# PaulMullowney/hypre

Measured on AMD Instinct MI355X. Metric: BoomerAMG V-cycle DOF/s (256^3 7-pt Laplacian per GPU, l1-Jacobi V(1,1), fp64), higher is better.
Workload: dtype f64; 1 GPU; 256x256x256 7-pt Laplacian, 1 rank(s) 1x1x1, PMIS + ext+i(4) + l1-Jacobi V(1,1); transport=none, replicated_from_level=-1, coarse_tail_graph_from_level=-1, coarse_tail_graph_nodes=0, one_workgroup_tail_from_level=6, levels=9

## Files before the change

### hypre_amd/binding.py

```python
import ctypes as C
import os

import numpy as np

HERE = os.path.dirname(os.path.abspath(__file__))
LIB_PATH = os.environ.get("HYPRE_AMD_LIB") or os.path.join(HERE, "lib", "libhypre_amd.so")

HYPRE_MEMORY_HOST = 0
HYPRE_MEMORY_DEVICE = 1

Int = C.c_int
BigInt = C.c_longlong
Real = C.c_double
IntP = C.POINTER(C.c_int)
BigIntP = C.POINTER(C.c_longlong)
RealP = C.POINTER(C.c_double)


class HypreAmdError(RuntimeError):
    pass


class CSRMatrix(C.Structure):
    _fields_ = [("i", IntP), ("j", IntP), ("big_j", BigIntP), ("num_rows", Int), ("num_cols", Int),
# ... 19 lines not shown
class ParCSRMatrix(C.Structure):
    _fields_ = [("comm", Int), ("global_num_rows", BigInt), ("global_num_cols", BigInt),
                ("global_num_rownnz", BigInt), ("num_nonzeros", BigInt), ("d_num_nonzeros", Real),
                ("first_row_index", BigInt), ("first_col_diag", BigInt), ("last_row_index", BigInt),
                ("last_col_diag", BigInt), ("diag", C.POINTER(CSRMatrix)), ("offd", C.POINTER(CSRMatrix)),
                ("diagT", C.POINTER(CSRMatrix)), ("offdT", C.POINTER(CSRMatrix)), ("col_map_offd", BigIntP),
                ("device_col_map_offd", BigIntP), ("row_starts", BigInt * 2), ("col_starts", BigInt * 2),
                ("comm_pkg", C.POINTER(CommPkg)), ("comm_pkgT", C.POINTER(CommPkg)), ("owns_data", Int),
                ("rowindices", BigIntP), ("rowvalues", RealP), ("getrowactive", Int),
                ("assumed_partition", C.c_void_p), ("owns_assumed_partition", Int), ("proc_ordering", IntP),
                ("bdiag_size", Int), ("bdiaginv", RealP), ("bdiaginv_comm_pkg", C.c_void_p),
                ("soc_diag_j", IntP), ("soc_offd_j", IntP)]


class ParVector(C.Structure):
    _fields_ = [("comm", Int), ("global_size", BigInt), ("first_index", BigInt), ("last_index", BigInt),
                ("partitioning", BigInt * 2), ("actual_local_size", Int), ("local_vector", C.POINTER(Vector)),
                ("owns_data", Int), ("all_zeros", Int), ("assumed_partition", C.c_void_p)]


class IJMatrix(C.Structure):
    _fields_ = [("comm", Int), ("row_partitioning", BigInt * 2), ("col_partitioning", BigInt * 2),
                ("object_type", Int), ("object", C.c_void_p), ("translator", C.c_void_p),
                ("assumed_part", C.c_void_p), ("assemble_flag", Int), ("global_first_row", BigInt),
                ("global_first_col", BigInt), ("global_num_rows", BigInt), ("global_num_cols", BigInt),
                ("omp_flag", Int), ("print_level", Int)]


class IJVector(C.Structure):
    _fields_ = [("comm", Int), ("partitioning", BigInt * 2), ("num_components", Int), ("object_type", Int),
                ("object", C.c_void_p), ("translator", C.c_void_p), ("assumed_part", C.c_void_p),
                ("global_first_row", BigInt), ("global_num_rows", BigInt), ("print_level", Int)]


HYPRE_PARCSR = 5555


class IntArray(C.Structure):
    _fields_ = [("data", IntP), ("size", Int), ("memory_location", Int)]


class ErrorStruct(C.Structure):
    _fields_ = [("error_flag", Int), ("temp_error_flag", Int), ("print_to_memory", Int), ("verbosity", Int),
                ("memory", C.c_char_p), ("mem_sz", Int), ("msg_sz", Int)]


EXCHANGE_FN = C.CFUNCTYPE(C.c_int, C.c_void_p, C.c_int, IntP, C.POINTER(C.c_void_p), C.POINTER(C.c_size_t),
                          C.c_int, IntP, C.POINTER(C.c_void_p), C.POINTER(C.c_size_t), C.c_int, C.c_void_p)
ALLREDUCE_FN = C.CFUNCTYPE(C.c_int, C.c_void_p, RealP, C.c_int, C.c_int, C.c_void_p)
ALLGATHER_FN = C.CFUNCTYPE(C.c_int, C.c_void_p, C.c_void_p, C.c_void_p, C.c_size_t)
BARRIER_FN = C.CFUNCTYPE(C.c_int, C.c_void_p)
DESTROY_FN = C.CFUNCTYPE(None, C.c_void_p)


class CommOps(C.Structure):
    _fields_ = [("ctx", C.c_void_p), ("rank", C.c_int), ("size", C.c_int), ("exchange", EXCHANGE_FN),
                ("allreduce_sum", ALLREDUCE_FN), ("allgather", ALLGATHER_FN), ("barrier", BARRIER_FN),
                ("destroy", DESTROY_FN), ("device_buffers", C.c_int)]


CSRp = C.POINTER(CSRMatrix)
Vecp = C.POINTER(Vector)
ParCSRp = C.POINTER(ParCSRMatrix)
ParVecp = C.POINTER(ParVector)

PROTOTYPES = {
    "hypre_error_handler": (None, [C.c_char_p, Int, Int, C.c_char_p]),
    "HYPRE_GetError": (Int, []),
    "HYPRE_CheckError": (Int, [Int, Int]),
    "HYPRE_ClearError": (Int, [Int]),
    "HYPRE_ClearAllErrors": (Int, []),
    "HYPRE_GetErrorArg": (Int, []),
    "hypre_amd_LastErrorMessage": (C.c_char_p, []),
    "HYPRE_Initialize": (Int, []),
    "hypre_amd_HostCpuShare": (Int, []),
    "hypre_amd_SetHostThreads": (Int, [Int]),
    "HYPRE_Finalize": (Int, []),
    "HYPRE_SetMemoryLocation": (Int, [Int]),
    "HYPRE_GetMemoryLocation": (Int, [IntP]),
    "HYPRE_SetExecutionPolicy": (Int, [Int]),
    "HYPRE_GetExecutionPolicy": (Int, [IntP]),
    "hypre_amd_DeviceAvailable": (Int, []),
    "hypre_SetSyncCudaCompute": (Int, [Int]),
    "hypre_GetSyncCudaCompute": (Int, [IntP]),
    "hypre_SyncComputeStream": (Int, []),
    "hypre_amd_ByteCounters": (Int, [C.POINTER(C.c_double), C.POINTER(C.c_double), Int]),
    "hypre_amd_ComputeStream": (C.c_void_p, []),
    "hypre_amd_CommStream": (C.c_void_p, []),
    "hypre_amd_EventTimerStart": (Int, []),
    "hypre_amd_EventTimerStopMs": (Real, []),
    "hypre_MAlloc": (C.c_void_p, [C.c_size_t, Int]),
    "hypre_CAlloc": (C.c_void_p, [C.c_size_t, C.c_size_t, Int]),
    "hypre_Free": (None, [C.c_void_p, Int]),
    "hypre_Memcpy": (None, [C.c_void_p, C.c_void_p, C.c_size_t, Int, Int]),
    "hypre_Memset": (None, [C.c_void_p, Int, C.c_size_t, Int]),
    "hypre_GetExecPolicy1": (Int, [Int]),
    "hypre_GetExecPolicy2": (Int, [Int, Int]),
    "hypre_IntArrayCreate": (C.POINTER(IntArray), [Int]),
    "hypre_IntArrayInitialize_v2": (Int, [C.POINTER(IntArray), Int]),
    "hypre_IntArrayDestroy": (Int, [C.POINTER(IntArray)]),
    "hypre_amd_CommCreate": (Int, [C.POINTER(CommOps)]),
    "hypre_amd_CommDestroy": (Int, [Int]),
    "hypre_amd_RCCLGetUniqueId": (Int, [C.c_void_p]),
    "hypre_amd_CommCreateRCCL": (Int, [C.c_void_p, C.c_int, C.c_int]),
    "hypre_amd_CommCreateStreamStaged": (Int, [Int]),
    "hypre_MPI_Comm_rank": (Int, [Int, IntP]),
    "hypre_MPI_Comm_size": (Int, [Int, IntP]),
    "hypre_amd_CommSelfTest": (Int, [Int, Int]),
    "hypre_MPI_Barrier": (Int, [Int]),
    "hypre_amd_CommCounters": (Int, [BigIntP, BigIntP, Int]),
    "hypre_amd_CommSetTiming": (Int, [Int]),
    "hypre_amd_CommSetTag": (Int, [Int]),
    "hypre_amd_CommExposedTimes": (Int, [Int, IntP, IntP, RealP, RealP, RealP]),
    "hypre_amd_CommBytes": (Int, [C.POINTER(C.c_longlong), C.POINTER(C.c_longlong)]),
    "hypre_amd_ParCSRMatrixHaloInfo": (Int, [ParCSRp, C.POINTER(C.c_int), C.POINTER(C.c_int), C.POINTER(C.c_int), C.POINTER(C.c_int)]),
    "hypre_CSRMatrixCreate": (CSRp, [Int, Int, Int]),
    "hypre_CSRMatrixInitialize_v2": (Int, [CSRp, Int, Int]),
    "hypre_CSRMatrixInitialize": (Int, [CSRp]),
    "hypre_CSRMatrixDestroy": (Int, [CSRp]),
    "hypre_CSRMatrixSetRownnz": (Int, [CSRp]),
    "hypre_CSRMatrixMigrate": (Int, [CSRp, Int]),
    "hypre_CSRMatrixClone_v2": (CSRp, [CSRp, Int, Int]),
    "hypre_CSRMatrixTranspose": (Int, [CSRp, C.POINTER(CSRp), Int]),
    "hypre_CSRMatrixReorder": (Int, [CSRp]),
    "hypre_SeqVectorCreate": (Vecp, [Int]),
    "hypre_SeqMultiVectorCreate": (Vecp, [Int, Int]),
    "hypre_SeqVectorInitialize_v2": (Int, [Vecp, Int]),
    "hypre_SeqVectorInitialize": (Int, [Vecp]),
    "hypre_SeqVectorDestroy": (Int, [Vecp]),
    "hypre_SeqVectorMigrate": (Int, [Vecp, Int]),
    "hypre_SeqVectorCloneDeep_v2": (Vecp, [Vecp, Int]),
    "hypre_SeqVectorCloneDeep": (Vecp, [Vecp]),
    "hypre_CSRMatrixMatvecOutOfPlace": (Int, [Real, CSRp, Vecp, Real, Vecp, Vecp, Int]),
    "hypre_CSRMatrixMatvec": (Int, [Real, CSRp, Vecp, Real, Vecp]),
    "hypre_CSRMatrixMatvecT": (Int, [Real, CSRp, Vecp, Real, Vecp]),
    "hypre_CSRMatrixMatvecDevice": (Int, [Int, Real, CSRp, Vecp, Real, Vecp, Vecp, Int]),
    "hypre_CSRMatrixSpMVDevice": (Int, [Int, Real, CSRp, Vecp, Real, Vecp, Int]),
    "hypre_amd_CSRMatrixInvalidatePlan": (Int, [CSRp]),
    "hypre_amd_CSRMatrixVerifyPlan": (Int, [CSRp]),
    "hypre_amd_CSRMatrixSetImmutable": (Int, [CSRp, Int]),
    "hypre_amd_CSRMatrixPlanForm": (Int, [CSRp]),
    "hypre_amd_PlanTestFailAlloc": (Int, [Int, Int]),
    "hypre_amd_SetMixedPrecisionValues": (Int, [Int]),
    "hypre_amd_SpmvSetRowSlices": (Int, [Int]),
    "hypre_amd_SpmvSetFusedMultivectors": (Int, [Int]),
    "hypre_amd_SpmvFusedMultivectorLaunches": (Int, []),
    "hypre_amd_CSRMatrixPlanRowSlices": (Int, [CSRp, IntP, IntP]),
    "hypre_amd_CSRMatrixSortRows": (Int, [CSRp, Int]),
    "hypre_amd_SpmvSetBandPolicy": (Int, [Int, Int, Int]),
    "hypre_amd_SpmvSetVariant": (Int, [Int, Int]),
    "hypre_amd_CSRMatrixPlanInfo": (Int, [CSRp, IntP, IntP]),
    "hypre_amd_CSRMatrixPlanStaging": (Int, [CSRp, IntP, RealP]),
    "hypre_amd_SpmvSetValueCodes": (Int, [Int]),
    "hypre_amd_SpmvSetSliceForm": (Int, [Int]),
    "hypre_amd_CSRMatrixPlanSliceForm": (Int, [CSRp]),
    "hypre_amd_SpmvSetSliceClasses": (Int, [Int]),
    "hypre_amd_CSRMatrixPlanSliceClasses": (Int, [CSRp]),
    "hypre_amd_CSRMatrixPlanSliceClassHistogram": (Int, [CSRp, C.POINTER(Int), C.POINTER(Int), C.POINTER(BigInt)]),
    "hypre_amd_CSRMatrixPlanValueCodes": (Int, [CSRp]),
    "hypre_SeqVectorSetConstantValues": (Int, [Vecp, Real]),
    "hypre_SeqVectorCopy": (Int, [Vecp, Vecp]),
    "hypre_SeqVectorScale": (Int, [Real, Vecp]),
    "hypre_SeqVectorAxpy": (Int, [Real, Vecp, Vecp]),
    "hypre_SeqVectorAxpyz": (Int, [Real, Vecp, Real, Vecp, Vecp]),
    "hypre_SeqVectorInnerProd": (Real, [Vecp, Vecp]),
    "hypre_SeqVectorElmdivpy": (Int, [Vecp, Vecp, Vecp]),
    "hypre_SeqVectorElmdivpyMarked": (Int, [Vecp, Vecp, Vecp, IntP, Int]),
    "hypre_SeqVectorSetConstantValuesDevice": (Int, [Vecp, Real]),
    "hypre_SeqVectorScaleDevice": (Int, [Real, Vecp]),
    "hypre_SeqVectorAxpyDevice": (Int, [Real, Vecp, Vecp]),
    "hypre_SeqVectorAxpyzDevice": (Int, [Real, Vecp, Real, Vecp, Vecp]),
    "hypre_SeqVectorInnerProdDevice": (Real, [Vecp, Vecp]),
    "hypre_SeqVectorElmdivpyDevice": (Int, [Vecp, Vecp, Vecp, IntP, Int]),
    "hypreDevice_IVAXPY": (Int, [Int, RealP, RealP, RealP]),
    "hypreDevice_IVAXPYMarked": (Int, [Int, RealP, RealP, RealP, IntP, Int]),
    "hypreDevice_DiagScaleVector2": (Int, [Int, Int, RealP, RealP, Real, RealP, RealP, Int]),
    "hypre_ParCSRMatrixCreate": (ParCSRp, [Int, BigInt, BigInt, BigIntP, BigIntP, Int, Int, Int]),
    "hypre_ParCSRMatrixInitialize_v2": (Int, [ParCSRp, Int]),
    "hypre_ParCSRMatrixDestroy": (Int, [ParCSRp]),
    "hypre_ParCSRMatrixMigrate": (Int, [ParCSRp, Int]),
    "hypre_ParCSRMatrixClone_v2": (ParCSRp, [ParCSRp, Int, Int]),
    "hypre_ParCSRMatrixSetNumNonzeros": (Int, [ParCSRp]),
    "hypre_ParCSRMatrixSetDNumNonzeros": (Int, [ParCSRp]),
    "hypre_amd_ParCSRMatrixKeepTranspose": (Int, [ParCSRp]),
    "hypre_ParVectorCreate": (ParVecp, [Int, BigInt, BigIntP]),
    "hypre_ParMultiVectorCreate": (ParVecp, [Int, BigInt, BigIntP, Int]),
    "hypre_ParCSRDiagScaleVector": (Int, [ParCSRp, ParVecp, ParVecp]),
    "hypre_ParVectorInitialize_v2": (Int, [ParVecp, Int]),
    "hypre_ParVectorInitialize": (Int, [ParVecp]),
    "hypre_ParVectorDestroy": (Int, [ParVecp]),
    "hypre_ParVectorSetLocalSize": (Int, [ParVecp, Int]),
    "hypre_ParVectorMigrate": (Int, [ParVecp, Int]),
    "hypre_MatvecCommPkgCreate": (Int, [ParCSRp]),
    "hypre_MatvecCommPkgDestroy": (Int, [C.POINTER(CommPkg)]),
    "hypre_ParCSRCommPkgUpdateVecStarts": (Int, [C.POINTER(CommPkg), Int, Int, Int]),
    "hypre_ParCSRCommPkgCreate_core": (Int, [Int, BigIntP, BigInt, BigIntP, Int, Int, IntP, C.POINTER(IntP),
                                             C.POINTER(IntP), IntP, C.POINTER(IntP), C.POINTER(IntP),
                                             C.POINTER(IntP)]),
    "hypre_ParCSRCommHandleCreate_v2": (C.c_void_p, [Int, C.POINTER(CommPkg), Int, C.c_void_p, Int, C.c_void_p]),
    "hypre_ParCSRCommHandleCreate": (C.c_void_p, [Int, C.POINTER(CommPkg), C.c_void_p, C.c_void_p]),
    "hypre_ParCSRCommHandleDestroy": (Int, [C.c_void_p]),
    "hypre_ParCSRMatrixMatvecOutOfPlace": (Int, [Real, ParCSRp, ParVecp, Real, ParVecp, ParVecp]),
    "hypre_ParCSRMatrixMatvec": (Int, [Real, ParCSRp, ParVecp, Real, ParVecp]),
    "hypre_ParCSRMatrixMatvecT": (Int, [Real, ParCSRp, ParVecp, Real, ParVecp]),
    "hypre_ParCSRMatrixMatvecOutOfPlaceDevice": (Int, [Real, ParCSRp, ParVecp, Real, ParVecp, ParVecp]),
    "hypre_ParCSRMatrixMatvecTDevice": (Int, [Real, ParCSRp, ParVecp, Real, ParVecp]),
    "HYPRE_ParCSRMatrixMatvec": (Int, [Real, ParCSRp, ParVecp, Real, ParVecp]),
    "hypre_ParVectorSetConstantValues": (Int, [ParVecp, Real]),
    "hypre_ParVectorSetZeros": (Int, [ParVecp]),
    "hypre_ParVectorCopy": (Int, [ParVecp, ParVecp]),
    "hypre_ParVectorScale": (Int, [Real, ParVecp]),
    "hypre_ParVectorAxpy": (Int, [Real, ParVecp, ParVecp]),
    "hypre_ParVectorAxpyz": (Int, [Real, ParVecp, Real, ParVecp, ParVecp]),
    "hypre_ParVectorInnerProd": (Real, [ParVecp, ParVecp]),
    "hypre_ParVectorElmdivpy": (Int, [ParVecp, ParVecp, ParVecp]),
    "hypre_ParVectorElmdivpyMarked": (Int, [ParVecp, ParVecp, ParVecp, IntP, Int]),
    "GenerateLaplacian": (ParCSRp, [Int, BigInt, BigInt, BigInt, Int, Int, Int, Int, Int, Int, RealP]),
    "GenerateLaplacian27pt": (ParCSRp, [Int, BigInt, BigInt, BigInt, Int, Int, Int, Int, Int, Int, RealP]),
    "GenerateDifConv": (ParCSRp, [Int, BigInt, BigInt, BigInt, Int, Int, Int, Int, Int, Int, RealP]),
    "GenerateVarDifConv": (ParCSRp, [Int, BigInt, BigInt, BigInt, Int, Int, Int, Int, Int, Int, Real, C.POINTER(ParVecp)]),
    "GenerateRotate7pt": (ParCSRp, [Int, BigInt, BigInt, Int, Int, Int, Int, Real, Real]),
    "GenerateSysLaplacian": (ParCSRp, [Int, BigInt, BigInt, BigInt, Int, Int, Int, Int, Int, Int, Int, RealP, RealP]),
    "hypre_amd_CSRMatrixFromArrays": (CSRp, [Int, Int, Int, IntP, IntP, RealP, Int]),
    "hypre_amd_SeqVectorFromArray": (Vecp, [Int, RealP, Int]),
    "hypre_amd_SeqVectorToArray": (Int, [Vecp, RealP]),
    "hypre_amd_CopyToHost": (Int, [C.c_void_p, C.c_void_p, C.c_size_t, Int]),
    "hypre_amd_ParCSRMatrixFromArrays": (ParCSRp, [Int, BigInt, BigInt, BigIntP, BigIntP, Int, BigIntP, IntP, IntP,
                                                   RealP, IntP, IntP, RealP, Int]),
    "hypre_amd_ParVectorFromArray": (ParVecp, [Int, BigInt, BigIntP, RealP, Int]),
    "hypre_amd_ParVectorToArray": (Int, [ParVecp, RealP]),
    "HYPRE_IJMatrixRead": (Int, [C.c_char_p, Int, Int, C.POINTER(C.POINTER(IJMatrix))]),
    "HYPRE_IJMatrixPrint": (Int, [C.POINTER(IJMatrix), C.c_char_p]),
    "HYPRE_IJMatrixGetObject": (Int, [C.POINTER(IJMatrix), C.POINTER(C.c_void_p)]),
    "HYPRE_IJMatrixDestroy": (Int, [C.POINTER(IJMatrix)]),
    "hypre_ParCSRMatrixPrintIJ": (Int, [ParCSRp, Int, Int, C.c_char_p]),
    "HYPRE_IJVectorRead": (Int, [C.c_char_p, Int, Int, C.POINTER(C.POINTER(IJVector))]),
    "HYPRE_IJVectorPrint": (Int, [C.POINTER(IJVector), C.c_char_p]),
    "HYPRE_IJVectorGetObject": (Int, [C.POINTER(IJVector), C.POINTER(C.c_void_p)]),
    "HYPRE_IJVectorDestroy": (Int, [C.POINTER(IJVector)]),
    "hypre_amd_IJMatrixWrap": (C.POINTER(IJMatrix), [ParCSRp]),
    "hypre_amd_IJVectorWrap": (C.POINTER(IJVector), [ParVecp]),
}

_lib = None


def load_library(build_if_missing=False):
    global _lib
    if _lib is not None:
        return _lib
    if not os.path.exists(LIB_PATH):
        if build_if_missing:
            from . import build as _b
            _b.build()
        else:
            raise HypreAmdError("HIP library %s is missing — run `python -m hypre_amd.build` "
                                "(there is no fallback implementation)" % LIB_PATH)
    lib = C.CDLL(LIB_PATH, mode=C.RTLD_GLOBAL)
    from . import parcsr_ls_binding as _ls
    for table in (PROTOTYPES, _ls.PROTOTYPES):
        for name, (res, args) in table.items():
            fn = getattr(lib, name)
            fn.restype = res
            fn.argtypes = args
    _lib = lib
    return lib


class _LazyLib:
    def __getattr__(self, name):
        return getattr(load_library(), name)


lib = _LazyLib()


def check():
    L = load_library()
    flag = L.HYPRE_GetError()
    if flag:
        msg = L.hypre_amd_LastErrorMessage().decode()
        L.HYPRE_ClearAllErrors()
        raise HypreAmdError("hypre error flag 0x%x: %s" % (flag, msg))


def _ip(a):
    return a.ctypes.data_as(IntP)


def _bp(a):
    return a.ctypes.data_as(BigIntP)


def _rp(a):
    return a.ctypes.data_as(RealP)


def csr_from_scipy(A, location=HYPRE_MEMORY_DEVICE):
    A = A.tocsr()
    ii = np.ascontiguousarray(A.indptr, dtype=np.int32)
    jj = np.ascontiguousarray(A.indices, dtype=np.int32)
    aa = np.ascontiguousarray(A.data, dtype=np.float64)
    m = lib.hypre_amd_CSRMatrixFromArrays(A.shape[0], A.shape[1], int(A.nnz), _ip(ii), _ip(jj), _rp(aa), location)
    check()
    return m

# ... 104 lines not shown
```

### hypre_amd/csrc/internal.hpp

```cpp
#pragma once

#include <hip/hip_runtime.h>
#include <cstdio>
#include <cstdlib>
#include <cstring>
#include <cstdint>
#include <vector>

#include "HYPRE_amd_utilities.h"
#include "hypre_amd_seq_mv.h"
#include "hypre_amd_comm.h"
#include "hypre_amd_parcsr_mv.h"

#define HIP_CHECK(call)                                                          \
   do {                                                                          \
      hipError_t e_ = (call);                                                    \
      if (e_ != hipSuccess) {                                                    \
         char msg_[512];                                                         \
         snprintf(msg_, sizeof(msg_), "HIP error %d (%s) in %s", (int) e_,       \
                  hipGetErrorString(e_), #call);                                 \
         hypre_error_handler(__FILE__, __LINE__, HYPRE_ERROR_GENERIC, msg_);     \
      }                                                                          \
   } while (0)

#define HYPRE_AMD_REQUIRE_DEVICE(loc, what)                                      \
   do {                                                                          \
      if ((loc) != HYPRE_MEMORY_DEVICE) {                                        \
         hypre_error_w_msg(HYPRE_ERROR_GENERIC,                                  \
                           what ": operand is not in device memory; host "       \
                           "execution is not part of this library");             \
         return hypre_error_flag;                                                \
      }                                                                          \
   } while (0)

namespace hamd {

struct Handle
{
   bool                  device_ok      = false;
   bool                  device_probed  = false;
   hipStream_t           compute_stream = nullptr;
   hipStream_t           comm_stream    = nullptr;
   int                   sync_compute   = 1;
   HYPRE_MemoryLocation  memory_location = HYPRE_MEMORY_DEVICE;
   HYPRE_ExecutionPolicy exec_policy     = HYPRE_EXEC_DEVICE;
   double               *d_reduce      = nullptr;
   size_t                d_reduce_len  = 0;
   double               *h_reduce      = nullptr;
   int                   num_cus       = 256;
   int                   gs_threads    = 1;
   bool                  fp32_values   = false;
   double                bytes_csr     = 0.0;
   double                bytes_stream  = 0.0;
};
Handle &handle();
inline void account_bytes(double csr, double stream) { Handle &h = handle(); h.bytes_csr += csr; h.bytes_stream += stream; }
inline void account_bytes(double b) { account_bytes(b, b); }
const hypre_amd_CommOps *comm_ops(MPI_Comm comm);
bool    ensure_device();
int     host_cpu_share();
hipStream_t stream();
void    maybe_sync();
double *reduce_scratch(size_t n);

#ifndef HYPRE_AMD_SPMV_TILE_NNZ
#define HYPRE_AMD_SPMV_TILE_NNZ 2048
#endif
#ifndef HYPRE_AMD_SPMV_WG
#define HYPRE_AMD_SPMV_WG 256
#endif
constexpr int SPMV_TILE    = HYPRE_AMD_SPMV_TILE_NNZ;
constexpr int SPMV_MAXROW  = 1024;
constexpr int SPMV_THREADS = HYPRE_AMD_SPMV_WG;
static_assert(SPMV_TILE == 8 * SPMV_THREADS, "a lane streams two quads of the tile");

struct SpmvPlan
{
   const HYPRE_Int     *i = nullptr;
   const HYPRE_Int     *j = nullptr;
   const HYPRE_Complex *a = nullptr;
   int   num_rows = 0, num_cols = 0, nnz = 0;
   int   max_row_nnz = 0;
   int   max_tile_rows = 0;
   int   num_tiles = 0;
   int  *d_tile_row = nullptr;
   int  *d_tile_k   = nullptr;
   int  *d_tile_perm = nullptr;
   int   band = 0;
   int   prod_elems = 0;
   bool  tiled = false;
   hypre_CSRMatrix *AT = nullptr;
   hypre_CSRMatrix *Lstrict = nullptr;
   float *a32 = nullptr;
   unsigned char *d_codes = nullptr;
   double        *d_dict = nullptr, *d_dict32 = nullptr;
   int            ndict = 0;
   int       sl_w = 0, sl_rows = 0, sl_k = 0;
   int       sl_wc = 0, sl_wl = 0;
   int       sl_blocks = 0, sl_launch_units = 0;
   int      *d_sl_cnt = nullptr, *d_sl_desc = nullptr;
   int      *d_sl_k0 = nullptr, *d_sl_fp = nullptr;
   int      *d_sl_perm = nullptr;
   unsigned *d_sl_data = nullptr;
   unsigned char *d_sl_cls = nullptr;
   unsigned      *d_sl_tab = nullptr;
   int           *d_sl_toff = nullptr;
   int            sl_classes = 0;
   long long      sl_class_total = 0;
   bool has_slice_form() const { return d_sl_data != nullptr || d_sl_cls != nullptr; }
   int             rs_w = 0, rs_rows = 0, rs_kp = 0;
   int             rs_blocks = 0, rs_units = 0;
   int            *d_rs_desc = nullptr;
   int            *d_rs_perm = nullptr;
   int            *d_rs_hdr = nullptr;
   unsigned       *d_rs_meta = nullptr;
   double         *d_rs_val = nullptr;
   float          *d_rs_val32 = nullptr;
   unsigned       *d_rs_idx = nullptr;
   int            *d_xs_cnt = nullptr;
   int            *d_xs_desc = nullptr;
   unsigned short *d_lidx   = nullptr;
   int             xs_tiles = 0;
   int             xs_max_units = 0;
   int             xs_launch_units = 0;
   int            *d_tile_fp = nullptr;
   int            *h_stale = nullptr;
   int            *d_stale = nullptr;
   unsigned        launches = 0;
   unsigned long long checksum = 0;
   bool            has_checksum = false;
   bool            owned = false;
};
void mark_owned(const hypre_CSRMatrix *A, bool on = true);
bool is_owned(const hypre_CSRMatrix *A);
bool plan_verify(hypre_CSRMatrix *A);
enum PlanAllocSite { PLAN_SITE_TILES = 1, PLAN_SITE_XS = 2, PLAN_SITE_CODES = 3, PLAN_SITE_SLICE = 4, PLAN_SITE_ROWSLICE = 5, PLAN_SITE_SLICE_CLASSES = 6,
                     PLAN_SITE_MV_LEVELS = 7 };
bool plan_alloc(void **ptr, size_t bytes, int site);
void plan_free(void *ptr);
inline void verify_par_plans(hypre_ParCSRMatrix *A)
{
   if (!A) { return; }
   if (A->diag && A->diag->memory_location == HYPRE_MEMORY_DEVICE) { (void) plan_verify(A->diag); }
   if (A->offd && A->offd->memory_location == HYPRE_MEMORY_DEVICE) { (void) plan_verify(A->offd); }
}
unsigned long long device_csr_checksum(const int *Ai, const int *Aj, const double *Aa, int n, int nnz, hipStream_t s);
void bump_plan_generation();
constexpr int MATRIX_FP_WORDS = 16;
struct MatrixWatch
{
   unsigned long long *d_fp = nullptr;
   int *h_stale = nullptr, *d_stale = nullptr;
};
void watch_record(MatrixWatch &w, const hypre_CSRMatrix *A, bool with_values, hipStream_t s);
void watch_check(const MatrixWatch &w, const hypre_CSRMatrix *A, bool with_values, hipStream_t s);
bool watch_flagged(const MatrixWatch &w);
void watch_release(MatrixWatch &w);
int *take_stale_slot(int **device_view);
void give_stale_slot(int *slot);
void launch_matrix_fingerprint(const int *Ai, const int *Aj, const double *Aa, int n, int nnz, unsigned long long *fp, int *stale,
                               int record, hipStream_t s);
unsigned long long plan_generation();
bool plan_is_stale(const hypre_CSRMatrix *A);
void launch_build_fp(const HYPRE_Int *Aj, int nnz, int num_tiles, int *fp, hipStream_t s);
SpmvPlan *get_plan(hypre_CSRMatrix *A);
hypre_CSRMatrix *strict_lower_of(hypre_CSRMatrix *A);
void      drop_plan(hypre_CSRMatrix *A);
const float *fp32_values_of(hypre_CSRMatrix *A);
void      set_strict_lower(hypre_CSRMatrix *A, hypre_CSRMatrix *L);

enum SpmvOp
{
   OP_AXPBY   = 0,
   OP_JACOBI  = 1,
   OP_JACOBI_CF = 2,
   OP_TSGS    = 3,
   OP_JACOBI_MAP = 4,
   OP_AXPBY_DIV = 5,
   OP_RESID_RD = 6,
   OP_TSGS_FIRST = 7
};

struct SpmvArgs
{
   const HYPRE_Int     *Ai;
   const HYPRE_Int     *Aj;
   const HYPRE_Complex *Aa;
   const float         *Aa32;
   const unsigned char *Ac8;
   const double        *dict;
   int                  ndict;
   int                  dict_rounded;
   const HYPRE_Complex *x;
   const HYPRE_Complex *b;
   HYPRE_Complex       *y;
   HYPRE_Complex       *aux;
   const HYPRE_Complex *d;
   const HYPRE_Int     *marker;
   int                  marker_val;
   HYPRE_Complex        alpha, beta;
   HYPRE_Complex        scale2;
   int                  fill;
   int                  row_offset;
   int                  last_quad;
   int                  x_last;
   int                  reduce_w;
   int                  gather_t;
   int                  xcd_map;
   const int           *tile_perm;
   const int           *tile_fp;
   int                 *stale;
   const int           *rowmap;
   int                  variant;
   int                  use_rs;
   unsigned             rot;
   int                  nnz;
};
void spmv_default_flags(SpmvArgs &a);

void launch_spmv(const SpmvPlan *plan, const SpmvArgs &args, SpmvOp op, hipStream_t s);
bool spmv_with_scaled_quotient(hypre_CSRMatrix *M, const double *x, double *y, double w, const double *d, double *u);
bool launch_spmv_mv(const SpmvPlan *plan, const SpmvArgs &args, SpmvOp op, int nv, long xstride, long bstride, long ystride, long auxstride,
                    hipStream_t s);
struct MvStrides { long x, b, y, aux; };
void spmv_columns(HYPRE_Complex alpha, hypre_CSRMatrix *A, const double *x, size_t xstride, HYPRE_Complex beta, const double *b,
                  size_t bstride, double *y, size_t ystride, int nv);
void spmv_columns_jacobi(hypre_CSRMatrix *A, const double *f, size_t fstride, double w, const double *d, const double *u_in, size_t instride,
                         double *u_out, size_t outstride, int nv);
bool spmv_columns_scaled_quotient(hypre_CSRMatrix *M, const double *x, size_t xstride, double *y, size_t ystride, double w, const double *d,
                                  double *u, size_t ustride, int nv);
long &spmv_mv_launches();
bool &spmv_fused_multivectors();
void launch_spmv_rownnz(const HYPRE_Int *rownnz, int num_rownnz, const SpmvArgs &args, hipStream_t s);
void launch_spmv_allrows_update(int num_rows, const SpmvArgs &args, hipStream_t s);
bool device_value_codes(const double *Aa, size_t nnz, unsigned char **codes_out, double **dict_out, double **dict32_out, int *ndict_out,
                        hipStream_t s);
bool device_build_slice_form(SpmvPlan *p, const hypre_CSRMatrix *A, hipStream_t s);
bool device_build_row_slices(SpmvPlan *p, const hypre_CSRMatrix *A, hipStream_t s);
int  &spmv_row_slices();
bool &spmv_slice_classes();
bool &spmv_slice_form();
bool &spmv_value_codes();
void launch_build_tiles(const HYPRE_Int *Ai, int num_rows, int nnz, int num_tiles, int *d_tile_row,
                        int *d_tile_k, hipStream_t s);
void launch_build_xs(const HYPRE_Int *Aj, const int *d_tile_k, int num_tiles, int *xs_cnt, int *xs_desc, unsigned short *lidx,
                     hipStream_t s);
constexpr int SPMV_XS_SEGS = 48;
constexpr int SPMV_XS_CAP  = 4096;
int  device_max_row_nnz(const HYPRE_Int *Ai, int num_rows, hipStream_t s);
void sample_row_bands(const HYPRE_Int *Ai, const HYPRE_Int *Aj, int num_rows, int nsamples, int *host_out, hipStream_t s);

void launch_set(double *y, double v, size_t n, hipStream_t s);
void launch_copy(double *y, const double *x, size_t n, hipStream_t s);
void launch_scale(double *y, double a, size_t n, hipStream_t s);
void launch_axpy(double a, const double *x, double *y, size_t n, hipStream_t s);
void launch_axpyz(double a, const double *x, double b, const double *y, double *z, size_t n, hipStream_t s);
void launch_elmdivpy(const double *x, const double *d, double *y, const int *marker, int mval,
                     size_t n, hipStream_t s);
void launch_scaled_div(double w, const double *f, const double *d, double *u, const int *marker,
                       int mval, size_t n, hipStream_t s);
void launch_diag_first_scale(const int *Ai, const double *Aa, const double *y, double *x, size_t n, int nv, size_t ys, size_t xs, hipStream_t s);
void launch_scaled_recip(double w, const double *f, const double *d, double *z, size_t n, hipStream_t s);
void launch_diagscale2(const double *diag, const double *x, double beta, double *y, double *z,
                       int computeY, size_t n, hipStream_t s);
void launch_dot(const double *x, const double *y, size_t n, double *d_out, hipStream_t s);
void launch_gather(const double *x, const int *idx, double *out, size_t n, hipStream_t s);
void launch_scatter_add(const double *in, const int *idx, double *y, size_t n, hipStream_t s);
void launch_f64_to_f32(const double *x, float *y, size_t n, hipStream_t s);
void launch_transpose(const int *Ai, const int *Aj, const double *Aa, int nrows, int ncols, int nnz, int *Ti, int *tj, double *ta,
                      hipStream_t s);
void launch_scan_exclusive(int *data, int n, hipStream_t s);
void launch_sort_rows(const int *Ai, int *Aj, double *Aa, int n, int keep_first, hipStream_t s);
void preload_mc_kernels();
void prepare_mc_plan(hypre_CSRMatrix *A);
int  device_greedy_coloring(int n, const int *Ai, const int *Aj, const int *Ti, const int *Tj, int *color, int round_budget, hipStream_t s,
                            int *rounds_out = nullptr);
void device_color_order(int n, int C, const int *color, int **order_out, std::vector<int> &cstart, hipStream_t s);
void device_color_matrices(int n, int C, const int *color, const int *order, const std::vector<int> &cstart, const int *Ai, const int *Aj,
                           const double *Aa, int **ptr_out, int **Cj_out, double **Ca_out, std::vector<int> &slice0, std::vector<int> &slice_nnz,
                           hipStream_t s);
void launch_mc_diag(int n, const int *Ai, const double *Aa, double *d, hipStream_t s);
void launch_mc_rowinfo(int n, const int *order, const int *Ai, void *info, hipStream_t s);
void launch_mc_small_sweep_ahead(int num_colors, int direction, const int *cstart, const void *rowinfo, int nrows, const int *Aj,
                                 const double *Aa, const float *Aa32, int nnz_matrix, const double *f, const double *d, const int *marker,
                                 int marker_val, double w, double *u, int n, int nnz, int r_first, hipStream_t s);
void launch_mc_small_sweep(int num_colors, int direction, const int *cstart, const int *order, const int *Ai, const int *Aj,
                           const double *Aa, const float *Aa32, const double *f, const double *d, const int *marker, int marker_val,
                           double w, double *u, int n, int nnz, hipStream_t s);
void preload_cheby_kernels(); void preload_gs_kernels(); void preload_interp_kernels(); void preload_vector_kernels();
void preload_rap_kernels(); void preload_setup_kernels(); void preload_spmv_kernels();
void device_strength(int n, const int *Ai, const int *Aj, const double *Aa, double theta, double max_row_sum,
                     int **Si_out, int **Sj_out, int *nnz_out, hipStream_t s);
int  device_pmis(int n, const int *Si, const int *Sj, int snnz, unsigned seed, unsigned long long skip, int *CF, hipStream_t s);
int  device_coarse_numbering(int n, const int *CF, int *f2c, hipStream_t s);
bool device_l1_norms(int n, const int *Ai, const int *Aj, const double *Aa, int option, const int *cf, double *out, hipStream_t s);
bool device_rap(int nc, int ncP, int maxP, const int *Ri, const int *Rj, const double *Ra, const int *Ai, const int *Aj,
                const double *Aa, const int *Pi, const int *Pj, const double *Pa, int **Ci_out, int **Cj_out, double **Ca_out,
                int *nnz_out, hipStream_t s);
bool device_extpi(int n, const int *Ai, const int *Aj, const double *Aa, const int *Si, const int *Sj, const int *CF,
                  const int *f2c, double trunc_tol, int max_elmts, int first_rung, int **Pi_out, int **Pj_out, double **Pa_out,
                  int *nnz_out, hipStream_t s, int split = -1, int **Oi_out = nullptr, int **Oj_out = nullptr,
                  double **Oa_out = nullptr, int *onnz_out = nullptr);
void preload_dist_setup_kernels();
void device_extend_csr(int n, const int *Di, const int *Dj, const double *Da, const int *Oi, const int *Oj, const double *Oa, int ooff,
                       int ng, const int *Gi, const int *Gj, const double *Ga, int **Ei_out, int **Ej_out, double **Ea_out,
                       int *nnz_out, hipStream_t s);
void device_extract_rows(int filter, int tot, const int *d_elmts, const int *Di, const int *Dj, const double *Da,
                         const int *Oi, const int *Oj, const double *Oa, long long first_col, const long long *d_cmap, const int *CF,
                         std::vector<int> &hi, std::vector<long long> &hj, std::vector<double> &ha, hipStream_t s);
void device_extract_S_rows(int tot, const int *d_elmts, int n, const int *Si, const int *Sj, long long first_col, const long long *d_cmap,
                           const int *CFext, std::vector<int> &hi, std::vector<long long> &hj, hipStream_t s);
void device_split_strided(int n, int stride, int *len, int *nd, const int *sj, const double *sa, int split,
                          int **Di_out, int **Dj_out, double **Da_out, int *dnnz, int **Oi_out, int **Oj_out, double **Oa_out, int *onnz,
                          hipStream_t s);
void device_split_pattern(int n, const int *Si, const int *Sj, int split, int **Di_out, int **Dj_out, int *dnnz,
                          int **Oi_out, int **Oj_out, int *onnz, hipStream_t s);
void launch_mark_used(const int *j, size_t nnz, int *used, hipStream_t s);
void launch_renumber(int *j, size_t nnz, int split, const int *map, hipStream_t s);
void launch_gather_int(const int *x, const int *idx, int *out, size_t n, hipStream_t s);
bool device_l1_norms_blocks(int n, const int *Di, const int *Dj, const double *Da, const int *Oi, const int *Oj, const double *Oa,
                            int option, const int *cf, const int *cfo, double *out, hipStream_t s);
void device_strength_blocks(int n, const int *Di, const int *Dj, const double *Da, const int *Oi, const int *Oj, const double *Oa,
                            double theta, double max_row_sum, int **Si_out, int **Sj_out, int *nnz_out, hipStream_t s);
int  device_pmis_dist(int n, int nco, const int *Si, const int *Sj, int snnz, unsigned seed, unsigned long long skip,
                      hypre_ParCSRCommPkg *pkg, const int *d_elmts, const int *d_prev, MPI_Comm comm, int *CF, hipStream_t s);
bool device_rap_dist(bool direct, int nc, int square, int ncols_out, int maxP, int max_seed,
                     const int *Ri, const int *Rj, const double *Ra, const int *Ai, const int *Aj, const double *Aa,
                     const int *A2i, const int *A2j, const double *A2a, int a2_off, int nfine,
                     const int *Pi, const int *Pj, const double *Pa,
                     const int *Fi, const int *Fj, const int *Xi, const int *Xj, const double *Xa, int split,
                     int **Di_out, int **Dj_out, double **Da_out, int *dnnz, int **Oi_out, int **Oj_out, double **Oa_out, int *onnz,
                     hipStream_t s);
void launch_deinterleave(const double *in, double *out, int n, int nv, hipStream_t s);
void launch_interleave(const double *in, double *out, int n, int nv, hipStream_t s);
void launch_count_lower(const HYPRE_Int *Ai, const HYPRE_Int *Aj, int n, int *cnt, hipStream_t s);
void launch_fill_lower(const HYPRE_Int *Ai, const HYPRE_Int *Aj, const double *Aa, const HYPRE_Int *Li, HYPRE_Int *Lj,
                       double *La, int n, hipStream_t s);
void launch_pcg_update(double a, double na, const double *p, const double *s, double *x, double *r, size_t n,
                       double *d_out, hipStream_t stream);
void launch_pcg_direction(double beta, const double *s, double *p, size_t n, hipStream_t stream);
double global_sum(MPI_Comm comm, double v);
void   dev_allreduce_sum(MPI_Comm comm, double *d_buf, int n);
void   dev_global_sums(MPI_Comm comm, double *d_vals, int n, double *h_out);
void launch_scale_copy(double b, const double *x, double *y, size_t n, hipStream_t s);

}
```

### hypre_amd/csrc/seq_mv.cpp

```cpp
#include "internal.hpp"
#include <unordered_map>
#include <unordered_set>
#include <omp.h>
#include <algorithm>

using namespace hamd;

namespace hamd {

struct SpmvVariant { int variant; };
static SpmvVariant &spmv_variant()
{
   static SpmvVariant v = {-1};
   if (v.variant < 0)
   {
      const char *e = getenv("HYPRE_AMD_SPMV_VARIANT");
      v.variant = e ? atoi(e) : 2;
   }
   return v;
}

void spmv_default_flags(SpmvArgs &a)
{
   static int gt = -1, xcd = 8;
   if (gt < 0)
   {
      const char *e = getenv("HYPRE_AMD_SPMV_GT");
      gt = e ? atoi(e) : 1;
      e = getenv("HYPRE_AMD_SPMV_XCD");
      xcd = e ? atoi(e) : 8;
   }
   a.gather_t = gt; a.xcd_map = xcd;
   a.variant = spmv_variant().variant;
   { static int w = -1; if (w < 0) { const char *e = getenv("HYPRE_AMD_SPMV_REDUCE_W"); w = e ? atoi(e) : 0; } a.reduce_w = w; }
}

struct BandPolicy { int enabled, min_tiles, force; };
static BandPolicy &band_policy()
{
   static BandPolicy bp = {-1, 2048, 0};
   if (bp.enabled < 0)
   {
      const char *e = getenv("HYPRE_AMD_SPMV_BAND");
      bp.enabled = e ? atoi(e) : 1;
      if ((e = getenv("HYPRE_AMD_SPMV_BAND_MIN_TILES"))) { bp.min_tiles = atoi(e); }
      if ((e = getenv("HYPRE_AMD_SPMV_BAND_FORCE"))) { bp.force = atoi(e); }
   }
   return bp;
}

int g_fail_site = 0, g_fail_nth = 0;
bool plan_alloc(void **ptr, size_t bytes, int site)
{
   *ptr = nullptr;
   if (g_fail_site == site && g_fail_nth > 0 && --g_fail_nth == 0) { g_fail_site = 0; return false; }
   size_t free_b = 0, total_b = 0;
   if (bytes > ((size_t) 64 << 20))
   {
      if (hipMemGetInfo(&free_b, &total_b) != hipSuccess) { (void) hipGetLastError(); return false; }
      if (bytes > free_b / 2) { return false; }
   }
   if (hipMalloc(ptr, bytes ? bytes : 16) != hipSuccess) { (void) hipGetLastError(); *ptr = nullptr; return false; }
   return true;
}
void plan_free(void *ptr) { if (ptr) { HIP_CHECK(hipFree(ptr)); } }

static std::unordered_set<const hypre_CSRMatrix *> &owned_table()
{
   static std::unordered_set<const hypre_CSRMatrix *> t;
   return t;
}
void mark_owned(const hypre_CSRMatrix *A, bool on)
{
   if (!A) { return; }
   if (on) { owned_table().insert(A); } else { owned_table().erase(A); }
}
bool is_owned(const hypre_CSRMatrix *A) { return A && owned_table().count(A) != 0; }

static void build_band_placement(SpmvPlan *p, const hypre_CSRMatrix *A, hipStream_t s)
{
   const BandPolicy &bp = band_policy();
   if (!bp.enabled || p->num_tiles < bp.min_tiles || p->num_tiles < 8 || A->num_rows != A->num_cols) { return; }
   const int ns = 1024;
   std::vector<int> far((size_t) ns);
   sample_row_bands(A->i, A->j, A->num_rows, ns, far.data(), s);
   std::vector<int> sorted(far);
   std::sort(sorted.begin(), sorted.end());
   const int B = sorted[(size_t) ns / 2];
   int agree = 0;
   for (int f : far) { if (std::abs(f - B) * 50 <= B) { agree++; } }
   const long long rows_per_tile = std::max(1LL, (long long) A->num_rows / p->num_tiles);
   if (B <= 0 || agree * 10 < ns * 6 || 4LL * B > A->num_rows) { return; }
   if (!bp.force && (long long) B < 8 * 8 * rows_per_tile) { return; }
   std::vector<int> trow((size_t) p->num_tiles + 1);
   HIP_CHECK(hipMemcpyAsync(trow.data(), p->d_tile_row, sizeof(int) * ((size_t) p->num_tiles + 1), hipMemcpyDeviceToHost, s));
   HIP_CHECK(hipStreamSynchronize(s));
   std::vector<std::vector<int>> cls(8);
   for (int t = 0; t < p->num_tiles; t++)
   {
      const int c = (int) (((long long) (trow[(size_t) t] % B) * 8) / B);
      cls[(size_t) std::min(std::max(c, 0), 7)].push_back(t);
   }
   std::vector<int> perm((size_t) p->num_tiles, -1);
   std::vector<size_t> next(8, 0);
   std::vector<int> leftovers;
   for (int g = 0; g < p->num_tiles; g++)
   {
      const size_t c = (size_t) (g & 7);
      if (next[c] < cls[c].size()) { perm[(size_t) g] = cls[c][next[c]++]; }
   }
   for (size_t c = 0; c < 8; c++) { for (size_t k = next[c]; k < cls[c].size(); k++) { leftovers.push_back(cls[c][k]); } }
   size_t lo = 0;
   for (int g = 0; g < p->num_tiles; g++) { if (perm[(size_t) g] < 0) { perm[(size_t) g] = leftovers[lo++]; } }
   if (!plan_alloc((void **) &p->d_tile_perm, sizeof(int) * (size_t) p->num_tiles, PLAN_SITE_TILES)) { return; }
   HIP_CHECK(hipMemcpyAsync(p->d_tile_perm, perm.data(), sizeof(int) * (size_t) p->num_tiles, hipMemcpyHostToDevice, s));
   HIP_CHECK(hipStreamSynchronize(s));
   p->band = B;
}

constexpr int RP_CAP_HOST = 640;

static std::unordered_map<const hypre_CSRMatrix *, SpmvPlan *> &plan_table()
{
   static std::unordered_map<const hypre_CSRMatrix *, SpmvPlan *> t;
   return t;
}

static unsigned long long g_plan_generation = 1;
unsigned long long plan_generation() { return g_plan_generation; }
void bump_plan_generation() { g_plan_generation++; }

namespace {
struct StaleSlots
{
   std::vector<int *> pages;
   std::vector<int *> free_list;
   int used_in_last = 1024;
   int *take()
   {
      if (!free_list.empty()) { int *p = free_list.back(); free_list.pop_back(); *p = 0; return p; }
      if (used_in_last >= 1024)
      {
         int *page = nullptr;
         if (hipHostMalloc((void **) &page, sizeof(int) * 1024, hipHostMallocMapped) != hipSuccess) { (void) hipGetLastError(); return nullptr; }
         memset(page, 0, sizeof(int) * 1024);
         pages.push_back(page);
         used_in_last = 0;
      }
      return pages.back() + used_in_last++;
   }
   void give(int *p) { if (p) { free_list.push_back(p); } }
};
StaleSlots &stale_slots() { static StaleSlots s; return s; }
}

int *take_stale_slot(int **device_view)
{
   int *h = stale_slots().take();
   int *d = nullptr;
   if (h && hipHostGetDevicePointer((void **) &d, h, 0) != hipSuccess) { (void) hipGetLastError(); d = nullptr; }
   if (!d) { stale_slots().give(h); h = nullptr; }
   if (device_view) { *device_view = d; }
   return h;
}
void give_stale_slot(int *slot) { stale_slots().give(slot); }

void watch_record(MatrixWatch &w, const hypre_CSRMatrix *A, bool with_values, hipStream_t s)
{
   watch_release(w);
   w.h_stale = take_stale_slot(&w.d_stale);
   if (!w.h_stale) { return; }
   HIP_CHECK(hipMalloc((void **) &w.d_fp, sizeof(unsigned long long) * MATRIX_FP_WORDS));
   launch_matrix_fingerprint(A->i, A->j, with_values ? A->data : nullptr, A->num_rows, A->num_nonzeros, w.d_fp, w.d_stale, 1, s);
}
void watch_check(const MatrixWatch &w, const hypre_CSRMatrix *A, bool with_values, hipStream_t s)
{
   if (!w.d_fp) { return; }
   launch_matrix_fingerprint(A->i, A->j, with_values ? A->data : nullptr, A->num_rows, A->num_nonzeros, w.d_fp, w.d_stale, 0, s);
}
bool watch_flagged(const MatrixWatch &w) { return w.h_stale && __atomic_load_n(w.h_stale, __ATOMIC_RELAXED) != 0; }
void watch_release(MatrixWatch &w)
{
   if (w.d_fp) { HIP_CHECK(hipFree(w.d_fp)); }
   give_stale_slot(w.h_stale);
   w = MatrixWatch();
}

static void free_plan(SpmvPlan *p)
{
   if (!p) { return; }
   g_plan_generation++;
   if (p->d_tile_fp) { HIP_CHECK(hipFree(p->d_tile_fp)); }
   stale_slots().give(p->h_stale);
   if (p->d_tile_row) { HIP_CHECK(hipFree(p->d_tile_row)); }
   if (p->d_tile_k) { HIP_CHECK(hipFree(p->d_tile_k)); }
   if (p->d_tile_perm) { HIP_CHECK(hipFree(p->d_tile_perm)); }
   if (p->d_xs_cnt) { HIP_CHECK(hipFree(p->d_xs_cnt)); }
   if (p->d_xs_desc) { HIP_CHECK(hipFree(p->d_xs_desc)); }
   if (p->d_lidx) { HIP_CHECK(hipFree(p->d_lidx)); }
   if (p->a32) { HIP_CHECK(hipFree(p->a32)); }
   if (p->d_codes) { HIP_CHECK(hipFree(p->d_codes)); }
   if (p->d_dict) { HIP_CHECK(hipFree(p->d_dict)); }
   if (p->d_sl_cnt) { HIP_CHECK(hipFree(p->d_sl_cnt)); }
   if (p->d_sl_desc) { HIP_CHECK(hipFree(p->d_sl_desc)); }
   if (p->d_sl_k0) { HIP_CHECK(hipFree(p->d_sl_k0)); }
   if (p->d_sl_fp) { HIP_CHECK(hipFree(p->d_sl_fp)); }
   if (p->d_sl_perm) { HIP_CHECK(hipFree(p->d_sl_perm)); }
   if (p->d_sl_data) { HIP_CHECK(hipFree(p->d_sl_data)); }
   if (p->d_sl_cls) { HIP_CHECK(hipFree(p->d_sl_cls)); }
   if (p->d_sl_tab) { HIP_CHECK(hipFree(p->d_sl_tab)); }
   if (p->d_sl_toff) { HIP_CHECK(hipFree(p->d_sl_toff)); }
   for (void *q : {(void *) p->d_rs_desc, (void *) p->d_rs_perm, (void *) p->d_rs_hdr, (void *) p->d_rs_meta, (void *) p->d_rs_val,
                   (void *) p->d_rs_val32, (void *) p->d_rs_idx}) { plan_free(q); }
   if (p->AT) { hypre_CSRMatrixDestroy(p->AT); }
   if (p->Lstrict) { hypre_CSRMatrixDestroy(p->Lstrict); }
   delete p;
}

void drop_gs_schedule(const hypre_CSRMatrix *A);
void drop_mc_plan(const hypre_CSRMatrix *A);

void drop_plan(hypre_CSRMatrix *A)
{
   drop_gs_schedule(A);
   drop_mc_plan(A);
   auto &t = plan_table();
   auto it = t.find(A);
   if (it != t.end())
   {
      free_plan(it->second);
      t.erase(it);
   }
}

static bool build_tile_tables(SpmvPlan *p, const hypre_CSRMatrix *A, hipStream_t s)
{
   p->num_tiles = (int) (((long long) A->num_nonzeros + SPMV_TILE - 1) / SPMV_TILE);
   if (!plan_alloc((void **) &p->d_tile_row, sizeof(int) * (size_t) (p->num_tiles + 1), PLAN_SITE_TILES) ||
       !plan_alloc((void **) &p->d_tile_k, sizeof(int) * (size_t) (p->num_tiles + 1), PLAN_SITE_TILES))
   {
      plan_free(p->d_tile_row); plan_free(p->d_tile_k);
      p->d_tile_row = p->d_tile_k = nullptr;
      p->num_tiles = 0;
      return false;
   }
   p->prod_elems = SPMV_TILE + ((p->max_row_nnz + 3) & ~3) + 8;
   launch_build_tiles(A->i, A->num_rows, A->num_nonzeros, p->num_tiles, p->d_tile_row, p->d_tile_k, s);
   p->max_tile_rows = device_max_row_nnz(p->d_tile_row, p->num_tiles, s);
   p->h_stale = stale_slots().take();
   if (p->h_stale && hipHostGetDevicePointer((void **) &p->d_stale, p->h_stale, 0) != hipSuccess) { (void) hipGetLastError(); p->d_stale = nullptr; }
   if (!p->d_stale)
   {
      static int *sink = nullptr;
      if (!sink && hipMalloc((void **) &sink, sizeof(int)) != hipSuccess) { (void) hipGetLastError(); sink = nullptr; }
      if (sink) { HIP_CHECK(hipMemsetAsync(sink, 0, sizeof(int), s)); }
      p->d_stale = sink;
      stale_slots().give(p->h_stale); p->h_stale = nullptr;
   }
   return true;
}

static void build_staging(SpmvPlan *p, const hypre_CSRMatrix *A, hipStream_t s)
{
   if (spmv_value_codes() && p->d_stale) { device_value_codes(A->data, (size_t) A->num_nonzeros, &p->d_codes, &p->d_dict, &p->d_dict32, &p->ndict, s); }
   const int rs_mode = spmv_row_slices();
   if (!p->d_codes && (rs_mode >= 2 || (rs_mode == 1 && p->owned)) && device_build_row_slices(p, A, s)) { return; }
   if (!p->d_stale) { plan_free(p->d_codes); plan_free(p->d_dict); p->d_codes = nullptr; p->d_dict = p->d_dict32 = nullptr; p->ndict = 0; return; }
   const size_t nl = ((size_t) A->num_nonzeros + 15) & ~(size_t) 7;
   if (!plan_alloc((void **) &p->d_tile_fp, sizeof(int) * (size_t) p->num_tiles, PLAN_SITE_XS) ||
       !plan_alloc((void **) &p->d_xs_cnt, sizeof(int) * (size_t) p->num_tiles, PLAN_SITE_XS) ||
       !plan_alloc((void **) &p->d_xs_desc, sizeof(int) * (size_t) p->num_tiles * 2 * SPMV_XS_SEGS, PLAN_SITE_XS) ||
       !plan_alloc((void **) &p->d_lidx, sizeof(unsigned short) * nl, PLAN_SITE_XS))
   {
      plan_free(p->d_tile_fp); plan_free(p->d_xs_cnt); plan_free(p->d_xs_desc); plan_free(p->d_lidx);
      p->d_tile_fp = nullptr; p->d_xs_cnt = nullptr; p->d_xs_desc = nullptr; p->d_lidx = nullptr;
      plan_free(p->d_codes); plan_free(p->d_dict);
      p->d_codes = nullptr; p->d_dict = p->d_dict32 = nullptr; p->ndict = 0;
      return;
   }
   launch_build_fp(A->j, A->num_nonzeros, p->num_tiles, p->d_tile_fp, s);
   HIP_CHECK(hipMemsetAsync(p->d_lidx, 0, sizeof(unsigned short) * nl, s));
   launch_build_xs(A->j, p->d_tile_k, p->num_tiles, p->d_xs_cnt, p->d_xs_desc, p->d_lidx, s);
   std::vector<int> cnt((size_t) p->num_tiles);
   HIP_CHECK(hipMemcpyAsync(cnt.data(), p->d_xs_cnt, sizeof(int) * (size_t) p->num_tiles, hipMemcpyDeviceToHost, s));
   HIP_CHECK(hipStreamSynchronize(s));
   std::vector<int> cov;
   cov.reserve(cnt.size());
   for (int c : cnt) { if (c & 0xff) { p->xs_tiles++; p->xs_max_units = std::max(p->xs_max_units, c >> 8); cov.push_back(c >> 8); } }
   if (!cov.empty())
   {
      std::sort(cov.begin(), cov.end());
      static int pct = -1, verbose = 0;
      if (pct < 0)
      {
         const char *e = getenv("HYPRE_AMD_SPMV_XS_PCT");
         pct = e ? std::min(100, std::max(1, atoi(e))) : 99;
         verbose = getenv("HYPRE_AMD_PLAN_VERBOSE") != nullptr;
      }
      const int need = cov[(size_t) ((cov.size() - 1) * (size_t) pct / 100)];
      const int rows = p->max_tile_rows > 0 ? std::min(p->max_tile_rows, RP_CAP_HOST) : RP_CAP_HOST;
      const int other = 8 * (p->max_row_nnz > 12 ? ((std::min(rows, SPMV_THREADS) + 1) & ~1) : 0) + 4 * (rows + 4) + 64 +
                        (p->d_codes ? 8 * ((p->ndict + 1) & ~1) + 16 : 0);
      int units = p->xs_max_units;
      for (int wgs = 8; wgs >= 3; wgs--)
      {
         const int room = ((160 * 1024) / wgs) / 1280 * 1280;
         const int fit = (room - other) / 16;
         if (fit >= need) { units = std::min(fit, p->xs_max_units); break; }
      }
      p->xs_launch_units = std::max(units, need);
      if (verbose)
      {
         fprintf(stderr, "[plan] %d x %d, %d tiles: staged units p50 %d p90 %d p99 %d max %d -> launch %d (%d bytes of LDS)\n",
                 A->num_rows, A->num_cols, p->num_tiles, cov[cov.size() / 2], cov[(cov.size() - 1) * 9 / 10],
                 cov[(cov.size() - 1) * 99 / 100], cov.back(), p->xs_launch_units, 16 * p->xs_launch_units + other);
      }
   }
   p->prod_elems = std::max(p->prod_elems, 2 * p->xs_launch_units + 8);
   if (p->d_codes && spmv_slice_form()) { device_build_slice_form(p, A, s); }
}

SpmvPlan *get_plan(hypre_CSRMatrix *A)
{
   auto &t = plan_table();
   auto it = t.find(A);
   if (it != t.end())
   {
      SpmvPlan *p = it->second;
      const bool flagged = p->h_stale && __atomic_load_n(p->h_stale, __ATOMIC_RELAXED) != 0;
      if (!flagged && p->i == A->i && p->j == A->j && p->a == A->data && p->nnz == A->num_nonzeros &&
          p->num_rows == A->num_rows && p->num_cols == A->num_cols)
      {
         return p;
      }
      if (flagged)
      {
         hypre_error_w_msg(HYPRE_ERROR_GENERIC, "a kernel found its SpMV plan out of date (the matrix at this address is not the one the plan "
                                                "was built for, or its values changed without hypre_amd_CSRMatrixInvalidatePlan): the products "
                                                "since then are wrong; the plan is rebuilt");
         drop_gs_schedule(A);
         drop_mc_plan(A);
      }
      free_plan(p);
      t.erase(it);
   }
   SpmvPlan *p = new SpmvPlan();
   p->i = A->i; p->j = A->j; p->a = A->data;
   p->num_rows = A->num_rows; p->num_cols = A->num_cols; p->nnz = A->num_nonzeros;
   p->owned = is_owned(A);
   hipStream_t s = stream();
   if (A->num_rows > 0 && A->num_nonzeros > 0)
   {
      p->max_row_nnz = device_max_row_nnz(A->i, A->num_rows, s);
      const bool aligned = (((uintptr_t) A->j) & 15) == 0 && (((uintptr_t) A->data) & 15) == 0;
      p->tiled = aligned && p->max_row_nnz <= SPMV_MAXROW && build_tile_tables(p, A, s);
      if (p->tiled)
      {
         build_band_placement(p, A, s);
         if (spmv_variant().variant == 2) { build_staging(p, A, s); }
      }
      if (p->tiled && !p->owned)
      {
         p->checksum = device_csr_checksum(A->i, A->j, A->data, A->num_rows, A->num_nonzeros, s);
         p->has_checksum = true;
      }
   }
   t[A] = p;
   return p;
}

bool plan_verify(hypre_CSRMatrix *A)
{
   auto &t = plan_table();
   auto it = t.find(A);
   if (it == t.end()) { return true; }
   SpmvPlan *p = it->second;
   if (!p->has_checksum) { return true; }
   const bool same_arrays = p->i == A->i && p->j == A->j && p->a == A->data && p->nnz == A->num_nonzeros &&
                            p->num_rows == A->num_rows && p->num_cols == A->num_cols;
   if (same_arrays && device_csr_checksum(A->i, A->j, A->data, A->num_rows, A->num_nonzeros, stream()) == p->checksum) { return true; }
   drop_plan(A);
   return false;
}

bool &spmv_slice_form()
{
   static bool on = [] { const char *e = getenv("HYPRE_AMD_SPMV_SLICE_FORM"); return !(e && atoi(e) == 0); }();
   return on;
}

bool &spmv_slice_classes()
{
   static bool on = [] { const char *e = getenv("HYPRE_AMD_SPMV_SLICE_CLASSES"); return !(e && atoi(e) == 0); }();
   return on;
}

bool &spmv_fused_multivectors()
{
   static bool on = [] { const char *e = getenv("HYPRE_AMD_SPMV_FUSED_MV"); return !(e && atoi(e) == 0); }();
   return on;
}

bool &spmv_value_codes()
{
   static bool on = [] { const char *e = getenv("HYPRE_AMD_SPMV_VALUE_CODES"); return !(e && atoi(e) == 0); }();
   return on;
}

bool plan_is_stale(const hypre_CSRMatrix *A)
{
   auto &t = plan_table();
   auto it = t.find(A);
   return it != t.end() && it->second->h_stale && __atomic_load_n(it->second->h_stale, __ATOMIC_RELAXED) != 0;
}

const float *fp32_values_of(hypre_CSRMatrix *A)
{
   if (!A || A->num_nonzeros <= 0 || !A->data) { return nullptr; }
   SpmvPlan *p = get_plan(A);
   if (!p->a32)
   {
      HIP_CHECK(hipMalloc((void **) &p->a32, sizeof(float) * (((size_t) A->num_nonzeros + 3) & ~(size_t) 3)));
      launch_f64_to_f32(A->data, p->a32, (size_t) A->num_nonzeros, stream());
   }
   return p->a32;
}

void set_strict_lower(hypre_CSRMatrix *A, hypre_CSRMatrix *L)
{
   SpmvPlan *plan = get_plan(A);
   if (plan->Lstrict && plan->Lstrict != L) { hypre_CSRMatrixDestroy(plan->Lstrict); }
   plan->Lstrict = L;
}

hypre_CSRMatrix *strict_lower_of(hypre_CSRMatrix *A)
{
   SpmvPlan *plan = get_plan(A);
   if (plan->Lstrict) { return plan->Lstrict; }
   const int n = A->num_rows;
   hipStream_t s = stream();
   std::vector<int> cnt((size_t) std::max(n, 1)), off((size_t) n + 1, 0);
   int *d_cnt = hypre_TAlloc(int, (size_t) std::max(n, 1), HYPRE_MEMORY_DEVICE);
   launch_count_lower(A->i, A->j, n, d_cnt, s);
   HIP_CHECK(hipMemcpyAsync(cnt.data(), d_cnt, sizeof(int) * (size_t) n, hipMemcpyDeviceToHost, s));
   HIP_CHECK(hipStreamSynchronize(s));
   for (int i = 0; i < n; i++) { off[(size_t) i + 1] = off[(size_t) i] + cnt[(size_t) i]; }
   hypre_Free(d_cnt, HYPRE_MEMORY_DEVICE);
   hypre_CSRMatrix *L = hypre_CSRMatrixCreate(n, A->num_cols, off[(size_t) n]);
   hypre_CSRMatrixInitialize_v2(L, 0, HYPRE_MEMORY_DEVICE);
   hypre_TMemcpy(L->i, off.data(), HYPRE_Int, (size_t) n + 1, HYPRE_MEMORY_DEVICE, HYPRE_MEMORY_HOST);
   if (off[(size_t) n] > 0) { launch_fill_lower(A->i, A->j, A->data, L->i, L->j, L->data, n, s); }
   if (plan->owned) { mark_owned(L); }
   plan->Lstrict = L;
   return L;
}

bool spmv_with_scaled_quotient(hypre_CSRMatrix *M, const double *x, double *y, double w, const double *d, double *u)
{
   if (!M || M->num_rows <= 0 || M->num_nonzeros <= 0 || !d || !u || M->memory_location != HYPRE_MEMORY_DEVICE) { return false; }
   SpmvArgs a{};
   a.Ai = M->i; a.Aj = M->j; a.Aa = M->data; a.Aa32 = nullptr;
   a.x = x; a.b = nullptr; a.y = y; a.d = d; a.aux = u; a.marker = nullptr; a.marker_val = 0;
   a.alpha = 1.0; a.beta = 0.0; a.scale2 = w; a.fill = HYPRE_SPMV_FILL_WHOLE; a.row_offset = 0;
   spmv_default_flags(a);
   launch_spmv(get_plan(M), a, OP_AXPBY_DIV, stream());
   return true;
}
}

extern "C" HYPRE_Int hypre_amd_SpmvSetBandPolicy(HYPRE_Int enabled, HYPRE_Int min_tiles, HYPRE_Int force)
{
   hamd::BandPolicy &bp = hamd::band_policy();
   if (enabled >= 0) { bp.enabled = enabled; }
   if (min_tiles >= 0) { bp.min_tiles = min_tiles; }
   if (force >= 0) { bp.force = force; }
   return hypre_error_flag;
}

extern "C" HYPRE_Int hypre_amd_SpmvSetVariant(HYPRE_Int variant, HYPRE_Int unused)
{
   (void) unused;
   hamd::SpmvVariant &v = hamd::spmv_variant();
   if (variant >= 0) { v.variant = variant; }
   return hypre_error_flag;
}

extern "C" HYPRE_Int hypre_amd_SpmvSetValueCodes(HYPRE_Int on)
{
   if (on >= 0) { hamd::spmv_value_codes() = on != 0; }
   return hypre_error_flag;
}

extern "C" HYPRE_Int hypre_amd_SpmvSetSliceForm(HYPRE_Int on)
{
   if (on >= 0) { hamd::spmv_slice_form() = on != 0; }
   return hypre_error_flag;
}

extern "C" HYPRE_Int hypre_amd_SpmvSetSliceClasses(HYPRE_Int on)
{
   if (on >= 0) { hamd::spmv_slice_classes() = on != 0; }
   return hypre_error_flag;
}
extern "C" HYPRE_Int hypre_amd_CSRMatrixPlanSliceClasses(hypre_CSRMatrix *A)
{
   if (!A || A->memory_location != HYPRE_MEMORY_DEVICE) { return 0; }
   hamd::SpmvPlan *p = hamd::get_plan(A);
   return p->d_sl_cls ? p->sl_classes : 0;
}

extern "C" HYPRE_Int hypre_amd_CSRMatrixPlanSliceClassHistogram(hypre_CSRMatrix *A, HYPRE_Int *hist, HYPRE_Int *blocks, HYPRE_BigInt *total)
{
   if (!A || A->memory_location != HYPRE_MEMORY_DEVICE) { return 0; }
   hamd::SpmvPlan *p = hamd::get_plan(A);
   if (!p->d_sl_cls) { return 0; }
   std::vector<int> toff((size_t) p->sl_blocks + 1);
   HIP_CHECK(hipStreamSynchronize(hamd::stream()));
   HIP_CHECK(hipMemcpy(toff.data(), p->d_sl_toff, sizeof(int) * toff.size(), hipMemcpyDeviceToHost));
   if (hist)
   {
      for (int c = 0; c < 256; c++) { hist[c] = 0; }
      for (int b = 0; b < p->sl_blocks; b++) { hist[std::min(std::max(toff[(size_t) b + 1] - toff[(size_t) b], 0), 255)]++; }
   }
   if (blocks) { *blocks = p->sl_blocks; }
   if (total) { *total = (HYPRE_BigInt) p->sl_class_total; }
   return p->sl_classes;
}

extern "C" HYPRE_Int hypre_amd_SpmvSetRowSlices(HYPRE_Int mode)
{
   if (mode >= 0) { hamd::spmv_row_slices() = mode; }
   return hypre_error_flag;
}
extern "C" HYPRE_Int hypre_amd_CSRMatrixPlanRowSlices(hypre_CSRMatrix *A, HYPRE_Int *rows_per_block, HYPRE_Int *entries_per_lane)
{
   if (rows_per_block) { *rows_per_block = 0; }
   if (entries_per_lane) { *entries_per_lane = 0; }
   if (!A || A->memory_location != HYPRE_MEMORY_DEVICE) { return 0; }
   hamd::SpmvPlan *p = hamd::get_plan(A);
   if (!p->d_rs_val) { return 0; }
   if (rows_per_block) { *rows_per_block = p->rs_rows; }
   if (entries_per_lane) { *entries_per_lane = p->rs_kp; }
   return p->rs_w;
}

extern "C" HYPRE_Int hypre_amd_CSRMatrixPlanSliceForm(hypre_CSRMatrix *A)
{
   if (A->memory_location != HYPRE_MEMORY_DEVICE) { return 0; }
   hamd::SpmvPlan *p = hamd::get_plan(A);
   return p->has_slice_form() ? p->sl_w : 0;
}

extern "C" HYPRE_Int hypre_amd_CSRMatrixPlanValueCodes(hypre_CSRMatrix *A)
{
   if (A->memory_location != HYPRE_MEMORY_DEVICE) { return 0; }
   hamd::SpmvPlan *p = hamd::get_plan(A);
   return p->d_codes ? p->ndict : 0;
}

extern "C" HYPRE_Int hypre_amd_CSRMatrixPlanInfo(hypre_CSRMatrix *A, HYPRE_Int *num_tiles, HYPRE_Int *band)
{
   if (A->memory_location != HYPRE_MEMORY_DEVICE) { if (num_tiles) { *num_tiles = 0; } if (band) { *band = 0; } return 0; }
   hamd::SpmvPlan *p = hamd::get_plan(A);
   if (num_tiles) { *num_tiles = p->tiled ? p->num_tiles : 0; }
   if (band) { *band = p->band; }
   return p->d_tile_perm != nullptr;
}

extern "C" HYPRE_Int hypre_amd_CSRMatrixPlanStaging(hypre_CSRMatrix *A, HYPRE_Int *num_tiles, HYPRE_Real *mean_pieces)
{
   if (num_tiles) { *num_tiles = 0; }
   if (mean_pieces) { *mean_pieces = 0.0; }
   if (A->memory_location != HYPRE_MEMORY_DEVICE) { return 0; }
   hamd::SpmvPlan *p = hamd::get_plan(A);
   if (!p->tiled || !p->d_xs_cnt) { return 0; }
   std::vector<int> cnt((size_t) p->num_tiles);
   HIP_CHECK(hipStreamSynchronize(hamd::stream()));
   HIP_CHECK(hipMemcpy(cnt.data(), p->d_xs_cnt, sizeof(int) * (size_t) p->num_tiles, hipMemcpyDeviceToHost));
   long long staged = 0, pieces = 0;
   for (int c : cnt) { if (c & 0xff) { staged++; pieces += c & 0xff; } }
   if (num_tiles) { *num_tiles = p->num_tiles; }
   if (mean_pieces && staged) { *mean_pieces = (double) pieces / (double) staged; }
   return (HYPRE_Int) staged;
}

extern "C" HYPRE_Int hypre_amd_CSRMatrixSortRows(hypre_CSRMatrix *A, HYPRE_Int keep_first)
{
   HYPRE_AMD_REQUIRE_DEVICE(A->memory_location, "hypre_amd_CSRMatrixSortRows(A)");
   hamd::drop_plan(A);
   if (A->num_nonzeros > 0) { hamd::launch_sort_rows(A->i, A->j, A->data, A->num_rows, keep_first, hamd::stream()); }
   hamd::maybe_sync();
   return hypre_error_flag;
}

extern "C" HYPRE_Int hypre_amd_CSRMatrixInvalidatePlan(hypre_CSRMatrix *A)
{
   drop_plan(A);
   return hypre_error_flag;
}

extern "C" HYPRE_Int hypre_amd_CSRMatrixVerifyPlan(hypre_CSRMatrix *A)
{
   if (!A || A->memory_location != HYPRE_MEMORY_DEVICE) { return 1; }
   return hamd::plan_verify(A) ? 1 : 0;
}

extern "C" HYPRE_Int hypre_amd_CSRMatrixSetImmutable(hypre_CSRMatrix *A, HYPRE_Int on)
{
   if (!A) { hypre_error_in_arg(1); return hypre_error_flag; }
   if (hamd::is_owned(A) != (on != 0)) { drop_plan(A); hamd::mark_owned(A, on != 0); }
   return hypre_error_flag;
}

extern "C" HYPRE_Int hypre_amd_PlanTestFailAlloc(HYPRE_Int site, HYPRE_Int nth)
{
   const HYPRE_Int pending = hamd::g_fail_site ? hamd::g_fail_nth : 0;
   hamd::g_fail_site = nth > 0 ? site : 0;
   hamd::g_fail_nth = nth > 0 ? nth : 0;
   return pending;
}

extern "C" HYPRE_Int hypre_amd_SetMixedPrecisionValues(HYPRE_Int on)
{
   hamd::handle().fp32_values = on != 0;
   return hypre_error_flag;
}

extern "C" HYPRE_Int hypre_amd_CSRMatrixPlanForm(hypre_CSRMatrix *A)
{
   if (!A || A->memory_location != HYPRE_MEMORY_DEVICE) { return -1; }
   hamd::SpmvPlan *p = hamd::get_plan(A);
   if (!p->tiled) { return 0; }
   if (p->d_rs_val) { return 5; }
   if (!p->d_lidx) { return 1; }
   if (p->has_slice_form()) { return 4; }
   if (p->d_codes) { return 3; }
   return 2;
}

extern "C" {

hypre_CSRMatrix *hypre_CSRMatrixCreate(HYPRE_Int num_rows, HYPRE_Int num_cols, HYPRE_Int num_nonzeros)
{
   hypre_CSRMatrix *m = (hypre_CSRMatrix *) calloc(1, sizeof(hypre_CSRMatrix));
   mark_owned(m, false);
   m->num_rows = num_rows;
   m->num_cols = num_cols;
   m->num_nonzeros = num_nonzeros;
   m->num_rownnz = num_rows;
   m->owns_data = 1;
   m->memory_location = handle().memory_location;
   return m;
}

HYPRE_Int hypre_CSRMatrixInitialize_v2(hypre_CSRMatrix *m, HYPRE_Int bigInit, HYPRE_MemoryLocation loc)
{
   m->memory_location = loc;
   if (!m->data && m->num_nonzeros) { m->data = hypre_CTAlloc(HYPRE_Complex, m->num_nonzeros, loc); }
   if (!m->i) { m->i = hypre_CTAlloc(HYPRE_Int, m->num_rows + 1, loc); }
   if (bigInit)
   {
      if (!m->big_j && m->num_nonzeros) { m->big_j = hypre_CTAlloc(HYPRE_BigInt, m->num_nonzeros, loc); }
   }
   else
   {
      if (!m->j && m->num_nonzeros) { m->j = hypre_CTAlloc(HYPRE_Int, m->num_nonzeros, loc); }
   }
   return hypre_error_flag;
}

HYPRE_Int hypre_CSRMatrixInitialize(hypre_CSRMatrix *m)
{
   return hypre_CSRMatrixInitialize_v2(m, 0, m->memory_location);
}

HYPRE_Int hypre_CSRMatrixDestroy(hypre_CSRMatrix *m)
{
   if (!m) { return hypre_error_flag; }
   drop_plan(m);
   mark_owned(m, false);
   const HYPRE_MemoryLocation loc = m->memory_location;
   hypre_Free(m->rownnz, loc);
   if (m->owns_data)
   {
      hypre_Free(m->data, loc);
      hypre_Free(m->i, loc);
      hypre_Free(m->j, loc);
      hypre_Free(m->big_j, loc);
   }
   free(m);
   return hypre_error_flag;
}

HYPRE_Int hypre_CSRMatrixSetRownnz(hypre_CSRMatrix *m)
{
   const HYPRE_MemoryLocation loc = m->memory_location;
   const HYPRE_Int n = m->num_rows;
   std::vector<HYPRE_Int> hi;
   const HYPRE_Int *Ai = m->i;
   if (loc == HYPRE_MEMORY_DEVICE)
   {
      hi.resize((size_t) n + 1);
      hypre_TMemcpy(hi.data(), m->i, HYPRE_Int, n + 1, HYPRE_MEMORY_HOST, HYPRE_MEMORY_DEVICE);
      Ai = hi.data();
   }
   HYPRE_Int cnt = 0;
   for (HYPRE_Int r = 0; r < n; r++) { if (Ai[r + 1] > Ai[r]) { cnt++; } }
   hypre_Free(m->rownnz, loc);
   m->rownnz = nullptr;
   m->num_rownnz = cnt;
   if (cnt == 0 || cnt == n) { return hypre_error_flag; }
   std::vector<HYPRE_Int> list((size_t) cnt);
   cnt = 0;
   for (HYPRE_Int r = 0; r < n; r++) { if (Ai[r + 1] > Ai[r]) { list[(size_t) cnt++] = r; } }
   m->rownnz = hypre_TAlloc(HYPRE_Int, cnt, loc);
   hypre_TMemcpy(m->rownnz, list.data(), HYPRE_Int, cnt, loc, HYPRE_MEMORY_HOST);
   return hypre_error_flag;
}

static void migrate_array(void **p, size_t bytes, HYPRE_MemoryLocation from, HYPRE_MemoryLocation to)
{
   if (!*p) { return; }
   void *q = hypre_MAlloc(bytes ? bytes : 8, to);
   if (bytes) { hypre_Memcpy(q, *p, bytes, to, from); }
   hypre_Free(*p, from);
   *p = q;
}

HYPRE_Int hypre_CSRMatrixMigrate(hypre_CSRMatrix *A, HYPRE_MemoryLocation to)
{
   const HYPRE_MemoryLocation from = A->memory_location;
   if (from == to) { return hypre_error_flag; }
   drop_plan(A);
   migrate_array((void **) &A->i, sizeof(HYPRE_Int) * (size_t) (A->num_rows + 1), from, to);
   migrate_array((void **) &A->j, sizeof(HYPRE_Int) * (size_t) A->num_nonzeros, from, to);
   migrate_array((void **) &A->big_j, sizeof(HYPRE_BigInt) * (size_t) A->num_nonzeros, from, to);
   migrate_array((void **) &A->data, sizeof(HYPRE_Complex) * (size_t) A->num_nonzeros, from, to);
   if (A->rownnz) { migrate_array((void **) &A->rownnz, sizeof(HYPRE_Int) * (size_t) A->num_rownnz, from, to); }
   A->memory_location = to;
   return hypre_error_flag;
}

hypre_CSRMatrix *hypre_CSRMatrixClone_v2(hypre_CSRMatrix *A, HYPRE_Int copy_data, HYPRE_MemoryLocation loc)
{
   hypre_CSRMatrix *B = hypre_CSRMatrixCreate(A->num_rows, A->num_cols, A->num_nonzeros);
   hypre_CSRMatrixInitialize_v2(B, A->big_j != nullptr && A->j == nullptr, loc);
   const HYPRE_MemoryLocation src = A->memory_location;
   hypre_TMemcpy(B->i, A->i, HYPRE_Int, A->num_rows + 1, loc, src);
   if (A->j) { hypre_TMemcpy(B->j, A->j, HYPRE_Int, A->num_nonzeros, loc, src); }
   if (A->big_j && B->big_j) { hypre_TMemcpy(B->big_j, A->big_j, HYPRE_BigInt, A->num_nonzeros, loc, src); }
   if (copy_data && A->data) { hypre_TMemcpy(B->data, A->data, HYPRE_Complex, A->num_nonzeros, loc, src); }
   B->num_rownnz = A->num_rownnz;
   if (A->rownnz)
   {
      B->rownnz = hypre_TAlloc(HYPRE_Int, A->num_rownnz, loc);
      hypre_TMemcpy(B->rownnz, A->rownnz, HYPRE_Int, A->num_rownnz, loc, src);
   }
   return B;
}

HYPRE_Int hypre_CSRMatrixTranspose(hypre_CSRMatrix *A, hypre_CSRMatrix **AT_ptr, HYPRE_Int data)
{
   const HYPRE_MemoryLocation loc = A->memory_location;
   const HYPRE_Int nr = A->num_rows, nc = A->num_cols, nnz = A->num_nonzeros;
   if (loc == HYPRE_MEMORY_DEVICE)
   {
      hypre_CSRMatrix *AT = hypre_CSRMatrixCreate(nc, nr, nnz);
      const bool with_data = data && A->data;
      hypre_CSRMatrixInitialize_v2(AT, 0, loc);
      if (!with_data && AT->data) { hypre_Free(AT->data, loc); AT->data = nullptr; }
      launch_transpose(A->i, A->j, with_data ? A->data : nullptr, nr, nc, nnz, AT->i, AT->j, with_data ? AT->data : nullptr, stream());
      HIP_CHECK(hipStreamSynchronize(stream()));
      *AT_ptr = AT;
      return hypre_error_flag;
   }
   const HYPRE_Int *Ai = A->i, *Aj = A->j;
   const HYPRE_Complex *Aa = A->data;
   const bool with_data = data && A->data;
   std::vector<HYPRE_Int> ti((size_t) nc + 1, 0), tj((size_t) nnz);
   std::vector<HYPRE_Complex> ta(with_data ? (size_t) nnz : 0);
   int T = 1;
   if (nnz > (1 << 20))
   {
      T = std::min(omp_get_max_threads(), 16);
      while (T > 1 && (size_t) T * (size_t) nc > (size_t) 1 << 30) { T /= 2; }
   }
   if (T <= 1)
   {
// ... 528 lines not shown
```

### hypre_amd/csrc/spmv_kernels.hip

```cpp
#include "amg_internal.hpp"

namespace hamd {

typedef int    v4i __attribute__((ext_vector_type(4)));
typedef int    v2i __attribute__((ext_vector_type(2)));
typedef double v2d __attribute__((ext_vector_type(2)));
typedef float  v4f __attribute__((ext_vector_type(4)));

__device__ __forceinline__ double wave_sum64(double v)
{
#pragma unroll
   for (int off = 32; off > 0; off >>= 1) { v += __shfl_xor(v, off, 64); }
   return v;
}

template <int W>
__device__ __forceinline__ double subwave_sum(double v)
{
#pragma unroll
   for (int off = W / 2; off > 0; off >>= 1) { v += __shfl_xor(v, off, 64); }
   return v;
}

__device__ __forceinline__ bool fill_keep(int fill, int row, int col)
// ... 1229 lines not shown
{
   extern __shared__ __align__(16) unsigned char smem_raw[];
   double *xs = reinterpret_cast<double *>(smem_raw);
   const double *dictl = xs + stage_elems;
   unsigned *tabl = reinterpret_cast<unsigned *>(xs + stage_elems + ((p.ndict + 1) & ~1));

   const int block = block_of_workgroup(sl_perm, blocks);
   if (block < 0) { return; }

   const int tid = threadIdx.x, lane = tid & 63;
   const int wave = __builtin_amdgcn_readfirstlane(tid >> 6);
   constexpr int R = SPMV_THREADS / W;
   const int r = block * R + tid / W, sub = tid % W;
   SlLane<CLS, KP> me;
   sl_lane_load<CLS, W, KP>(me, st, p.Ai, block, wave, lane, tid, r, num_rows);
   const RowOps ops = load_row_ops<OP>(p, max(min(r, num_rows - 1), 0));
   const XPieces pc = wave_x_pieces(sl_desc, block, wave);
   const int k0 = sl_k0[block], k1b = sl_k0[block + 1], fp_plan = sl_fp[block];
   asm volatile("" :: "s"(sl_desc), "s"(sl_k0), "s"(sl_fp), "s"(CLS ? (const void *) st.toff : (const void *) st.data), "s"(st.tab), "s"(p.Ai) : "memory");
   stage_x_pieces<1>(p.x, 0, xs, 0, pc, lane);
   sl_lane_stage<CLS, KP>(me, st, wave, lane, tabl);
   stage_value_table(p.dict, p.ndict, dictl, wave, lane);
   const int q0 = min(max(k0, 0), nnz - 1), q1 = min(max(k0, 0) + 1, nnz - 1);
   const int fc0 = p.Aj[q0], fc1 = p.Aj[q1];
   const int ck = min(max(min(k0 + 8 * (int) ((4u * p.rot + (unsigned) wave) & 511u) + (lane & 7), k1b - 1), 0), nnz - 1);
   const double ckv = p.Aa[ck];
   const unsigned ckc = p.Ac8[ck];
   __syncthreads();

   const int mylen = sl_lane_words<CLS, W, KP>(me, tid, tabl);
   double sum = 0.0;
#pragma unroll
   for (int j = 0; j < KP; j++)
   {
      const unsigned code = (me.cw[j >> 2] >> (8 * (j & 3))) & 0xffu;
      const unsigned li = (me.lw[j >> 1] >> (16 * (j & 1))) & 0xffffu;
      {
#pragma clang fp contract(off)
         const double pr = dictl[code] * xs[li];
         if (j < mylen) { sum = sum + pr; }
      }
   }
   if (W == 2) { sum += __shfl_xor(sum, 1, 64); }
   {
      bool off = __double_as_longlong(dictl[ckc]) != __double_as_longlong(p.dict_rounded ? (double) (float) ckv : ckv);
      if (tid == 0) { off = off || fp_plan != plan_fingerprint(fc0, fc1) || me.rs != k0; }
      if (off) { mark_stale(p); }
   }
   if (r < num_rows && sub == 0) { row_epilogue<OP>(p, r, sum, ops); }
}
template <int OP, int W, int KP>
__global__ __launch_bounds__(SPMV_THREADS)
void spmv_sl_kernel(SpmvArgs p, const int *__restrict__ sl_cnt, const int *__restrict__ sl_desc, const int *__restrict__ sl_k0,
                    const int *__restrict__ sl_fp, const int *__restrict__ sl_perm, const unsigned *__restrict__ sl_data,
                    int blocks, int num_rows, int nnz, int stage_elems)
{
   const SlStream st = {sl_data, nullptr, nullptr, nullptr};
   spmv_sl_body<OP, W, KP, false>(p, sl_desc, sl_k0, sl_fp, sl_perm, st, blocks, num_rows, nnz, stage_elems);
}
template <int OP, int W, int KP>
__global__ __launch_bounds__(SPMV_THREADS)
void spmv_sl_kernel_cls(SpmvArgs p, const int *__restrict__ sl_desc, const int *__restrict__ sl_k0, const int *__restrict__ sl_fp,
                        const int *__restrict__ sl_perm, const unsigned char *__restrict__ sl_cls, const unsigned *__restrict__ sl_tab,
                        const int *__restrict__ sl_toff, int blocks, int num_rows, int nnz, int stage_elems)
{
   const SlStream st = {nullptr, sl_cls, sl_tab, sl_toff};
   spmv_sl_body<OP, W, KP, true>(p, sl_desc, sl_k0, sl_fp, sl_perm, st, blocks, num_rows, nnz, stage_elems);
}

template <int NV, int W, int KP, bool CLS, int OP>
__device__ __forceinline__
void spmv_sl_mv_body(const SpmvArgs &p, const int *__restrict__ sl_desc, const int *__restrict__ sl_k0,
                     const int *__restrict__ sl_fp, const int *__restrict__ sl_perm, const SlStream &st,
                     int blocks, int num_rows, int nnz, int stage_elems, MvStrides ms)
{
   extern __shared__ __align__(16) unsigned char smem_raw[];
   double *xs = reinterpret_cast<double *>(smem_raw);
   const double *dictl = xs + (size_t) NV * stage_elems;
   unsigned *tabl = reinterpret_cast<unsigned *>(xs + (size_t) NV * stage_elems + ((p.ndict + 1) & ~1));

   const int block = block_of_workgroup(sl_perm, blocks);
   if (block < 0) { return; }

   const int tid = threadIdx.x, lane = tid & 63;
   const int wave = __builtin_amdgcn_readfirstlane(tid >> 6);
   constexpr int R = SPMV_THREADS / W;
   const int r = block * R + tid / W, sub = tid % W;
   SlLane<CLS, KP> me;
   sl_lane_load<CLS, W, KP>(me, st, p.Ai, block, wave, lane, tid, r, num_rows);
   MvOps<NV> ops;
   mv_load_ops<NV, OP>(ops, p, max(min(r, num_rows - 1), 0), ms);
   const XPieces pc = wave_x_pieces(sl_desc, block, wave);
   const int k0 = sl_k0[block], k1b = sl_k0[block + 1], fp_plan = sl_fp[block];
   asm volatile("" :: "s"(sl_desc), "s"(sl_k0), "s"(sl_fp), "s"(CLS ? (const void *) st.toff : (const void *) st.data), "s"(st.tab), "s"(p.Ai) : "memory");
   sl_lane_stage<CLS, KP>(me, st, wave, lane, tabl);
   stage_x_pieces<NV>(p.x, ms.x, xs, stage_elems, pc, lane);
   stage_value_table(p.dict, p.ndict, dictl, wave, lane);
   const int q0 = min(max(k0, 0), nnz - 1), q1 = min(max(k0, 0) + 1, nnz - 1);
   const int fc0 = p.Aj[q0], fc1 = p.Aj[q1];
   const int ck = min(max(min(k0 + 8 * (int) ((4u * p.rot + (unsigned) wave) & 511u) + (lane & 7), k1b - 1), 0), nnz - 1);
   const double ckv = p.Aa[ck];
   const unsigned ckc = p.Ac8[ck];
   __syncthreads();

   const int mylen = sl_lane_words<CLS, W, KP>(me, tid, tabl);
   double sum[NV];
#pragma unroll
   for (int v = 0; v < NV; v++) { sum[v] = 0.0; }
#pragma unroll
   for (int j = 0; j < KP; j++)
   {
      const unsigned code = (me.cw[j >> 2] >> (8 * (j & 3))) & 0xffu;
      const unsigned li = (me.lw[j >> 1] >> (16 * (j & 1))) & 0xffffu;
      const double a = dictl[code];
#pragma unroll
      for (int v = 0; v < NV; v++)
      {
#pragma clang fp contract(off)
         const double pr = a * xs[v * stage_elems + li];
         if (j < mylen) { sum[v] = sum[v] + pr; }
      }
   }
   if (W == 2)
   {
#pragma unroll
      for (int v = 0; v < NV; v++) { sum[v] += __shfl_xor(sum[v], 1, 64); }
   }
   {
      bool off = __double_as_longlong(dictl[ckc]) != __double_as_longlong(ckv);
      if (tid == 0) { off = off || fp_plan != plan_fingerprint(fc0, fc1) || me.rs != k0; }
      if (off) { mark_stale(p); }
   }
   if (r < num_rows && sub == 0) { mv_epilogue<NV, OP>(p, r, sum, ops, ms); }
}
template <int NV, int W, int KP, int OP>
__global__ __launch_bounds__(SPMV_THREADS)
void spmv_sl_mv_kernel(SpmvArgs p, const int *__restrict__ sl_desc, const int *__restrict__ sl_k0,
                       const int *__restrict__ sl_fp, const int *__restrict__ sl_perm, const unsigned *__restrict__ sl_data,
                       int blocks, int num_rows, int nnz, int stage_elems, MvStrides ms)
{
   const SlStream st = {sl_data, nullptr, nullptr, nullptr};
   spmv_sl_mv_body<NV, W, KP, false, OP>(p, sl_desc, sl_k0, sl_fp, sl_perm, st, blocks, num_rows, nnz, stage_elems, ms);
}
template <int NV, int W, int KP, int OP>
__global__ __launch_bounds__(SPMV_THREADS)
void spmv_sl_mv_kernel_cls(SpmvArgs p, const int *__restrict__ sl_desc, const int *__restrict__ sl_k0, const int *__restrict__ sl_fp,
                           const int *__restrict__ sl_perm, const unsigned char *__restrict__ sl_cls, const unsigned *__restrict__ sl_tab,
                           const int *__restrict__ sl_toff, int blocks, int num_rows, int nnz, int stage_elems, MvStrides ms)
{
   const SlStream st = {nullptr, sl_cls, sl_tab, sl_toff};
   spmv_sl_mv_body<NV, W, KP, true, OP>(p, sl_desc, sl_k0, sl_fp, sl_perm, st, blocks, num_rows, nnz, stage_elems, ms);
}

__global__ void sl_block_starts_kernel(const int *__restrict__ Ai, int num_rows, int R, int blocks, int *__restrict__ k0)
{
   const int b = blockIdx.x * blockDim.x + threadIdx.x;
   if (b <= blocks) { k0[b] = Ai[min((long long) b * R, (long long) num_rows)]; }
}
__global__ void sl_fp_kernel(const int *__restrict__ Aj, const int *__restrict__ k0, int blocks, int nnz, int *__restrict__ fp)
{
   const int b = blockIdx.x * blockDim.x + threadIdx.x;
   if (b >= blocks) { return; }
   const int q0 = min(max(k0[b], 0), nnz - 1), q1 = min(max(k0[b], 0) + 1, nnz - 1);
   fp[b] = plan_fingerprint(Aj[q0], Aj[q1]);
}
template <int W>
__global__ __launch_bounds__(SPMV_THREADS)
void sl_pack_kernel(const int *__restrict__ Ai, const unsigned char *__restrict__ codes, const unsigned short *__restrict__ lidx,
                    int num_rows, int kper, int wc, int wl, unsigned *__restrict__ data)
{
   constexpr int R = SPMV_THREADS / W;
   const int block = blockIdx.x, tid = threadIdx.x, lane = tid & 63, wave = tid >> 6;
   const int r = block * R + tid / W, sub = tid % W;
   const int rs = r < num_rows ? Ai[r] : 0, re = r < num_rows ? Ai[r + 1] : 0;
   unsigned *out = data + ((size_t) (block * 4 + wave) * (size_t) (wc + wl)) * 64 + lane;
   for (int w = 0; w < wc; w++)
   {
      unsigned word = 0;
      for (int q = 0; q < 4; q++)
      {
         const int j = 4 * w + q, k = rs + sub + j * W;
         if (j < kper && k < re) { word |= (unsigned) codes[k] << (8 * q); }
      }
      out[w * 64] = word;
   }
   for (int w = 0; w < wl; w++)
   {
      unsigned word = 0;
      for (int q = 0; q < 2; q++)
      {
         const int j = 2 * w + q, k = rs + sub + j * W;
         if (j < kper && k < re) { word |= (unsigned) lidx[k] << (16 * q); }
      }
      out[(wc + w) * 64] = word;
   }
}

constexpr int SL_CLASS_CAP = 255;
static inline int sl_stage_elems_of(int units, bool classes) { return classes ? std::max(2 * units + 8, SPMV_THREADS) : 2 * units + 8; }
template <int W>
__device__ inline void sl_lane_tuple(const int *__restrict__ Ai, const unsigned *__restrict__ data, int num_rows, int wc, int wl,
                                     int block, int tid, unsigned *tup)
{
   constexpr int R = SPMV_THREADS / W;
   const int lane = tid & 63, wave = tid >> 6, t = tid / W, sub = tid % W;
   const int r = block * R + t;
   const int rs = r < num_rows ? Ai[r] : 0, re = r < num_rows ? Ai[r + 1] : 0;
   const int mylen = max((re - rs - sub + W - 1) / W, 0);
   const unsigned *sd = data + ((size_t) (block * 4 + wave) * (size_t) (wc + wl)) * 64 + lane;
   tup[0] = (unsigned) mylen;
   for (int w = 0; w < wc; w++) { tup[1 + w] = sd[w * 64]; }
   for (int w = 0; w < wl; w++)
   {
      const unsigned v = sd[(wc + w) * 64];
      const unsigned lo = 2 * w < mylen ? ((v & 0xffffu) - (unsigned) t) & 0xffffu : 0u;
      const unsigned hi = 2 * w + 1 < mylen ? ((v >> 16) - (unsigned) t) & 0xffffu : 0u;
      tup[1 + wc + w] = lo | (hi << 16);
   }
   for (int w = 1 + wc + wl; w < 16; w++) { tup[w] = 0u; }
}
template <int W>
__global__ __launch_bounds__(SPMV_THREADS)
void sl_classify_kernel(const int *__restrict__ Ai, const unsigned *__restrict__ data, int num_rows, int wc, int wl,
                        unsigned char *__restrict__ cls, int *__restrict__ ncls)
{
   __shared__ unsigned tupS[SPMV_THREADS][17];
   __shared__ int leader;
   const int block = blockIdx.x, tid = threadIdx.x;
   unsigned tup[16];
   sl_lane_tuple<W>(Ai, data, num_rows, wc, wl, block, tid, tup);
   for (int w = 0; w < 16; w++) { tupS[tid][w] = tup[w]; }
   int mine = -1, round = 0;
   while (true)
   {
      if (tid == 0) { leader = SPMV_THREADS; }
      __syncthreads();
      if (mine < 0) { atomicMin(&leader, tid); }
      __syncthreads();
      const int L = leader;
      if (L == SPMV_THREADS || round == SL_CLASS_CAP) { if (L != SPMV_THREADS) { round = SL_CLASS_CAP + 1; } break; }
      if (mine < 0)
      {
         bool eq = true;
         for (int w = 0; w < 16; w++) { eq = eq && tupS[L][w] == tup[w]; }
         if (eq) { mine = round; }
      }
      round++;
      __syncthreads();
   }
   cls[(size_t) block * SPMV_THREADS + tid] = (unsigned char) max(mine, 0);
   if (tid == 0) { ncls[block] = round; }
}
template <int W>
__global__ __launch_bounds__(SPMV_THREADS)
void sl_class_table_kernel(const int *__restrict__ Ai, const unsigned *__restrict__ data, int num_rows, int wc, int wl, int kper,
                           const unsigned char *__restrict__ cls, const int *__restrict__ toff, unsigned *__restrict__ tab)
{
   __shared__ int first[256];
   const int block = blockIdx.x, tid = threadIdx.x;
   first[tid] = SPMV_THREADS;
   __syncthreads();
   const int c = cls[(size_t) block * SPMV_THREADS + tid];
   atomicMin(&first[c], tid);
   __syncthreads();
   if (first[c] != tid) { return; }
   unsigned tup[16];
   sl_lane_tuple<W>(Ai, data, num_rows, wc, wl, block, tid, tup);
   unsigned *out = tab + ((size_t) toff[block] + (size_t) c) * (size_t) kper;
   for (int w = 0; w < kper; w++) { out[w] = tup[w]; }
}
static_assert(SPMV_THREADS == 256, "a class byte per lane of a 256-lane block; sl_class_table_kernel's first[]");

static bool device_build_slice_classes(SpmvPlan *p, const hypre_CSRMatrix *A, hipStream_t s)
{
   const int blocks = p->sl_blocks, kper = p->sl_k, wc = p->sl_wc, wl = p->sl_wl, n = A->num_rows;
   unsigned char *d_cls = nullptr;
   int *d_ncls = nullptr, *d_toff = nullptr;
   unsigned *d_tab = nullptr;
   auto fail = [&]() -> bool
   {
      HIP_CHECK(hipStreamSynchronize(s));
      for (void *q : {(void *) d_cls, (void *) d_ncls, (void *) d_toff, (void *) d_tab}) { plan_free(q); }
      return false;
   };
   if (!plan_alloc((void **) &d_cls, (size_t) blocks * SPMV_THREADS, PLAN_SITE_SLICE_CLASSES) ||
       !plan_alloc((void **) &d_ncls, sizeof(int) * (size_t) blocks, PLAN_SITE_SLICE_CLASSES) ||
       !plan_alloc((void **) &d_toff, sizeof(int) * ((size_t) blocks + 1), PLAN_SITE_SLICE_CLASSES)) { return fail(); }
   if (p->sl_w == 1) { hipLaunchKernelGGL((sl_classify_kernel<1>), dim3(blocks), dim3(SPMV_THREADS), 0, s, A->i, p->d_sl_data, n, wc, wl, d_cls, d_ncls); }
   else              { hipLaunchKernelGGL((sl_classify_kernel<2>), dim3(blocks), dim3(SPMV_THREADS), 0, s, A->i, p->d_sl_data, n, wc, wl, d_cls, d_ncls); }
   std::vector<int> ncls((size_t) blocks), toff((size_t) blocks + 1, 0);
   HIP_CHECK(hipMemcpyAsync(ncls.data(), d_ncls, sizeof(int) * (size_t) blocks, hipMemcpyDeviceToHost, s));
   HIP_CHECK(hipStreamSynchronize(s));
   int most = 0;
   long long total = 0;
   for (int b = 0; b < blocks; b++)
   {
      most = std::max(most, ncls[(size_t) b]);
      total += ncls[(size_t) b];
      if (total > 0x7fffffffLL / 16) { return fail(); }
      toff[(size_t) b + 1] = (int) total;
   }
   if (most < 1 || most > SL_CLASS_CAP) { return fail(); }
   if (8 * ((size_t) sl_stage_elems_of(p->sl_launch_units, true) + DICT_CAP) + 4 * (size_t) most * kper > 40 * 1024) { return fail(); }
   const double packed_bytes = 4.0 * (double) blocks * 4.0 * (wc + wl) * 64.0;
   const double class_bytes = (double) blocks * SPMV_THREADS + 4.0 * (double) total * kper + 4.0 * ((double) blocks + 1.0);
   if (class_bytes > 0.5 * packed_bytes) { return fail(); }
// ... 445 lines not shown
      }
      sum = wave_sum64(sum);
      if (lane == 0) { const RowOps o = load_row_ops<OP>(p, row); row_epilogue<OP>(p, row, sum, o); }
   }
}

__global__ __launch_bounds__(SPMV_THREADS)
void spmv_rownnz_kernel(SpmvArgs p, const int *__restrict__ rownnz, int num_rownnz)
{
   const int g   = (blockIdx.x * SPMV_THREADS + threadIdx.x) >> 3;
   const int sub = threadIdx.x & 7;
   double sum = 0.0;
   int row = 0;
   if (g < num_rownnz)
   {
      row = rownnz ? rownnz[g] : g;
      const int s = p.Ai[row], e = p.Ai[row + 1];
      for (int k = s + sub; k < e; k += 8)
      {
         const double v = p.Aa32 ? (double) p.Aa32[k] : p.Aa[k];
         sum += v * p.x[p.Aj[k]];
      }
   }
   sum = subwave_sum<8>(sum);
   if (g < num_rownnz && sub == 0)
   {
      if (p.marker && p.marker[row] != p.marker_val) { return; }
      double upd = p.alpha * sum;
      if (p.d) { upd /= p.d[row]; }
      p.y[row] += upd;
   }
}

__global__ void build_tiles_kernel(const int *__restrict__ Ai, int num_rows, int num_tiles,
                                   int *__restrict__ tile_row, int *__restrict__ tile_k)
{
   const int b = blockIdx.x * blockDim.x + threadIdx.x;
   if (b > num_tiles) { return; }
   if (b == num_tiles) { tile_row[b] = num_rows; tile_k[b] = Ai[num_rows]; return; }
   const long long target = (long long) b * SPMV_TILE;
   int lo = 0, hi = num_rows;
   while (lo < hi)
   {
      const int mid = (lo + hi) >> 1;
      if ((long long) Ai[mid] >= target) { hi = mid; } else { lo = mid + 1; }
   }
   tile_row[b] = lo;
   tile_k[b] = Ai[lo];
}

__global__ void max_row_nnz_kernel(const int *__restrict__ Ai, int num_rows, int *__restrict__ out)
{
   int m = 0;
   for (int r = blockIdx.x * blockDim.x + threadIdx.x; r < num_rows; r += gridDim.x * blockDim.x)
   {
      m = max(m, Ai[r + 1] - Ai[r]);
   }
#pragma unroll
   for (int off = 32; off > 0; off >>= 1) { m = max(m, __shfl_xor(m, off, 64)); }
   if ((threadIdx.x & 63) == 0) { atomicMax(out, m); }
}

__global__ void build_fp_kernel(const HYPRE_Int *__restrict__ Aj, int last_quad, int num_tiles, int *__restrict__ fp)
{
   const int t = blockIdx.x * blockDim.x + threadIdx.x;
   if (t >= num_tiles) { return; }
   const int ka = t * SPMV_TILE;
   const int c0 = Aj[min(ka + 5, last_quad)], c1 = Aj[min(ka + 1029, last_quad)];
   fp[t] = plan_fingerprint(c0, c1);
}
void launch_build_fp(const HYPRE_Int *Aj, int nnz, int num_tiles, int *fp, hipStream_t s)
{
   if (num_tiles <= 0) { return; }
   hipLaunchKernelGGL(build_fp_kernel, dim3((num_tiles + 255) / 256), dim3(256), 0, s, Aj, (nnz > 0 ? nnz - 1 : 0) & ~3, num_tiles, fp);
}

void launch_build_tiles(const HYPRE_Int *Ai, int num_rows, int nnz, int num_tiles, int *d_tile_row,
                        int *d_tile_k, hipStream_t s)
{
   (void) nnz;
   const int n = num_tiles + 1;
   hipLaunchKernelGGL(build_tiles_kernel, dim3((n + 255) / 256), dim3(256), 0, s, Ai, num_rows,
                      num_tiles, d_tile_row, d_tile_k);
}

__global__ void sample_row_bands_kernel(const HYPRE_Int *__restrict__ Ai, const HYPRE_Int *__restrict__ Aj, int num_rows,
                                        int nsamples, int *__restrict__ out)
{
   const int t = blockIdx.x * blockDim.x + threadIdx.x;
   if (t >= nsamples) { return; }
   const int row = (int) ((long long) num_rows * t / nsamples);
   int far = 0;
   for (int k = Ai[row]; k < Ai[row + 1]; k++) { far = max(far, abs(Aj[k] - row)); }
   out[t] = far;
}

void sample_row_bands(const HYPRE_Int *Ai, const HYPRE_Int *Aj, int num_rows, int nsamples, int *host_out, hipStream_t s)
{
   int *d_out = reinterpret_cast<int *>(reduce_scratch(((size_t) nsamples + 1) / 2));
   hipLaunchKernelGGL(sample_row_bands_kernel, dim3((nsamples + 255) / 256), dim3(256), 0, s, Ai, Aj, num_rows, nsamples, d_out);
   HIP_CHECK(hipMemcpyAsync(host_out, d_out, sizeof(int) * (size_t) nsamples, hipMemcpyDeviceToHost, s));
   HIP_CHECK(hipStreamSynchronize(s));
}

int device_max_row_nnz(const HYPRE_Int *Ai, int num_rows, hipStream_t s)
{
   if (num_rows <= 0) { return 0; }
   int *d_out = reinterpret_cast<int *>(reduce_scratch(2));
   HIP_CHECK(hipMemsetAsync(d_out, 0, sizeof(int), s));
   int grid = (num_rows + 255) / 256;
   if (grid > 2048) { grid = 2048; }
   hipLaunchKernelGGL(max_row_nnz_kernel, dim3(grid), dim3(256), 0, s, Ai, num_rows, d_out);
   int h = 0;
   HIP_CHECK(hipMemcpyAsync(&h, d_out, sizeof(int), hipMemcpyDeviceToHost, s));
   HIP_CHECK(hipStreamSynchronize(s));
   return h;
}

__device__ __forceinline__ unsigned long long mix64(unsigned long long x)
{
   x ^= x >> 30; x *= 0xbf58476d1ce4e5b9ull; x ^= x >> 27; x *= 0x94d049bb133111ebull; x ^= x >> 31;
   return x;
}
__global__ __launch_bounds__(256)
void csr_checksum_kernel(const int *__restrict__ Ai, const int *__restrict__ Aj, const unsigned long long *__restrict__ Aa,
                         int n, int nnz, unsigned long long *out)
{
   unsigned long long acc = 0;
   const size_t stride = (size_t) gridDim.x * blockDim.x, t = (size_t) blockIdx.x * blockDim.x + threadIdx.x;
   for (size_t r = t; r <= (size_t) n; r += stride) { acc += mix64(((unsigned long long) r << 32) ^ (unsigned) Ai[r] ^ 0x9e3779b97f4a7c15ull); }
   for (size_t k = t; k < (size_t) nnz; k += stride)
   {
      acc += mix64(Aa[k] ^ mix64(((unsigned long long) k << 32) | (unsigned) Aj[k]));
   }
#pragma unroll
   for (int off = 32; off > 0; off >>= 1) { acc += __shfl_xor(acc, off, 64); }
   if ((threadIdx.x & 63) == 0) { atomicAdd(out, acc); }
}
unsigned long long device_csr_checksum(const int *Ai, const int *Aj, const double *Aa, int n, int nnz, hipStream_t s)
{
   unsigned long long *d_out = reinterpret_cast<unsigned long long *>(reduce_scratch(2));
   HIP_CHECK(hipMemsetAsync(d_out, 0, sizeof(unsigned long long), s));
   const size_t work = (size_t) std::max(nnz, n + 1);
   const int grid = (int) std::min<size_t>((work + 255) / 256, (size_t) 16 * handle().num_cus);
   hipLaunchKernelGGL(csr_checksum_kernel, dim3(std::max(grid, 1)), dim3(256), 0, s, Ai, Aj, reinterpret_cast<const unsigned long long *>(Aa), n, nnz, d_out);
   unsigned long long h = 0;
   HIP_CHECK(hipMemcpyAsync(&h, d_out, sizeof(h), hipMemcpyDeviceToHost, s));
   HIP_CHECK(hipStreamSynchronize(s));
   return h;
}

constexpr int DICT_SLOTS = 4 * DICT_CAP;
constexpr unsigned long long DICT_EMPTY = ~0ull;
__device__ __forceinline__ unsigned dict_hash(unsigned long long v)
{
   v ^= v >> 33; v *= 0xff51afd7ed558ccdull; v ^= v >> 29;
   return (unsigned) v & (DICT_SLOTS - 1);
}
__global__ __launch_bounds__(256)
void dict_collect_kernel(const unsigned long long *__restrict__ vals, size_t n, unsigned long long *table, int *count)
{
   unsigned long long last = DICT_EMPTY;
   for (size_t k = (size_t) blockIdx.x * blockDim.x + threadIdx.x; k < n; k += (size_t) gridDim.x * blockDim.x)
   {
      const unsigned long long v = vals[k];
      if (v == last) { continue; }
      if (v == DICT_EMPTY || __hip_atomic_load(count, __ATOMIC_RELAXED, __HIP_MEMORY_SCOPE_AGENT) > DICT_CAP)
      {
         __hip_atomic_store(count, DICT_CAP + 1, __ATOMIC_RELAXED, __HIP_MEMORY_SCOPE_AGENT);
         return;
      }
      unsigned slot = dict_hash(v);
      for (;;)
      {
         unsigned long long cur = __hip_atomic_load(table + slot, __ATOMIC_RELAXED, __HIP_MEMORY_SCOPE_AGENT);
         if (cur == DICT_EMPTY)
         {
            cur = atomicCAS(table + slot, DICT_EMPTY, v);
            if (cur == DICT_EMPTY) { atomicAdd(count, 1); break; }
         }
         if (cur == v) { break; }
         if (__hip_atomic_load(count, __ATOMIC_RELAXED, __HIP_MEMORY_SCOPE_AGENT) > DICT_CAP) { return; }
         slot = (slot + 1) & (DICT_SLOTS - 1);
      }
      last = v;
   }
}
__global__ __launch_bounds__(256)
void dict_encode_kernel(const unsigned long long *__restrict__ vals, size_t n, const unsigned long long *__restrict__ table,
                        const unsigned char *__restrict__ code_of_slot, unsigned char *__restrict__ codes)
{
   __shared__ unsigned long long t[DICT_SLOTS];
   __shared__ unsigned char c[DICT_SLOTS];
   for (int i = threadIdx.x; i < DICT_SLOTS; i += blockDim.x) { t[i] = table[i]; c[i] = code_of_slot[i]; }
   __syncthreads();
   for (size_t k = (size_t) blockIdx.x * blockDim.x + threadIdx.x; k < n; k += (size_t) gridDim.x * blockDim.x)
   {
      const unsigned long long v = vals[k];
      unsigned slot = dict_hash(v);
      while (t[slot] != v) { slot = (slot + 1) & (DICT_SLOTS - 1); }
      codes[k] = c[slot];
   }
}

bool device_value_codes(const double *Aa, size_t nnz, unsigned char **codes_out, double **dict_out, double **dict32_out, int *ndict_out,
                        hipStream_t s)
{
   *codes_out = nullptr; *dict_out = nullptr; *dict32_out = nullptr; *ndict_out = 0;
   if (nnz < 8) { return false; }
   unsigned long long *d_table = nullptr;
   if (!plan_alloc((void **) &d_table, sizeof(unsigned long long) * DICT_SLOTS + sizeof(int) * 4, PLAN_SITE_CODES)) { return false; }
   int *d_count = reinterpret_cast<int *>(d_table + DICT_SLOTS);
   HIP_CHECK(hipMemsetAsync(d_table, 0xff, sizeof(unsigned long long) * DICT_SLOTS, s));
   HIP_CHECK(hipMemsetAsync(d_count, 0, sizeof(int) * 4, s));
   const unsigned long long *bits = reinterpret_cast<const unsigned long long *>(Aa);
   int count = 0;
   const size_t head = std::min<size_t>(nnz, 16384);
   hipLaunchKernelGGL(dict_collect_kernel, dim3((unsigned) ((head + 255) / 256)), dim3(256), 0, s, bits, head, d_table, d_count);
   HIP_CHECK(hipMemcpyAsync(&count, d_count, sizeof(int), hipMemcpyDeviceToHost, s));
   HIP_CHECK(hipStreamSynchronize(s));
   if (count > DICT_CAP) { plan_free(d_table); return false; }
   int grid = (int) std::min<size_t>((nnz + 255) / 256, (size_t) 8 * handle().num_cus);
   if (nnz > head) { hipLaunchKernelGGL(dict_collect_kernel, dim3(grid), dim3(256), 0, s, bits, nnz, d_table, d_count); }
   std::vector<unsigned long long> table(DICT_SLOTS);
   HIP_CHECK(hipMemcpyAsync(&count, d_count, sizeof(int), hipMemcpyDeviceToHost, s));
   HIP_CHECK(hipMemcpyAsync(table.data(), d_table, sizeof(unsigned long long) * DICT_SLOTS, hipMemcpyDeviceToHost, s));
   HIP_CHECK(hipStreamSynchronize(s));
   if (count > DICT_CAP || count <= 0) { plan_free(d_table); return false; }
   std::vector<unsigned long long> vals;
   for (unsigned long long v : table) { if (v != DICT_EMPTY) { vals.push_back(v); } }
   std::sort(vals.begin(), vals.end());
   if ((int) vals.size() != count) { plan_free(d_table); hypre_error_w_msg(HYPRE_ERROR_GENERIC, "value table: count and contents disagree"); return false; }
   std::vector<unsigned char> code_of_slot(DICT_SLOTS, 0);
   for (int i = 0; i < DICT_SLOTS; i++)
   {
      if (table[(size_t) i] != DICT_EMPTY) { code_of_slot[(size_t) i] = (unsigned char) (std::lower_bound(vals.begin(), vals.end(), table[(size_t) i]) - vals.begin()); }
   }
   std::vector<double> dict(DICT_CAP, 0.0), dict32(DICT_CAP, 0.0);
   for (size_t i = 0; i < vals.size(); i++)
   {
      double d; memcpy(&d, &vals[i], sizeof(double));
      dict[i] = d; dict32[i] = (double) (float) d;
   }
   unsigned char *d_cos = nullptr, *d_codes = nullptr;
   double *d_dict = nullptr;
   const size_t ncodes = (nnz + 31) & ~(size_t) 15;
   if (!plan_alloc((void **) &d_cos, DICT_SLOTS, PLAN_SITE_CODES) || !plan_alloc((void **) &d_codes, ncodes, PLAN_SITE_CODES) ||
       !plan_alloc((void **) &d_dict, sizeof(double) * 2 * DICT_CAP, PLAN_SITE_CODES))
   {
      plan_free(d_cos); plan_free(d_codes); plan_free(d_dict); plan_free(d_table);
      return false;
   }
   HIP_CHECK(hipMemcpyAsync(d_cos, code_of_slot.data(), DICT_SLOTS, hipMemcpyHostToDevice, s));
   HIP_CHECK(hipMemcpyAsync(d_dict, dict.data(), sizeof(double) * DICT_CAP, hipMemcpyHostToDevice, s));
   HIP_CHECK(hipMemcpyAsync(d_dict + DICT_CAP, dict32.data(), sizeof(double) * DICT_CAP, hipMemcpyHostToDevice, s));
   HIP_CHECK(hipMemsetAsync(d_codes + (ncodes - 32), 0, 32, s));
   grid = (int) std::min<size_t>((nnz + 255) / 256, (size_t) 16 * handle().num_cus);
   hipLaunchKernelGGL(dict_encode_kernel, dim3(grid), dim3(256), 0, s, bits, nnz, d_table, d_cos, d_codes);
   HIP_CHECK(hipStreamSynchronize(s));
   plan_free(d_cos);
   plan_free(d_table);
   *codes_out = d_codes; *dict_out = d_dict; *dict32_out = d_dict + DICT_CAP; *ndict_out = count;
   return true;
}

static inline size_t tiled_lds_bytes(const SpmvPlan *plan, int &rowsum_elems, int &rp_cap)
{
   static int fit = -1;
   if (fit < 0) { const char *e = getenv("HYPRE_AMD_SPMV_LDSFIT"); fit = e ? atoi(e) : 1; }
   const int rows = (fit && plan->max_tile_rows > 0) ? plan->max_tile_rows : RP_CAP;
   rp_cap = rows < RP_CAP ? rows : RP_CAP;
   rowsum_elems = plan->max_row_nnz > 12 ? ((rows < SPMV_THREADS ? rows : SPMV_THREADS) + 1) & ~1 : 0;
   return sizeof(double) * (size_t) (plan->prod_elems + rowsum_elems) + sizeof(int) * (size_t) (rp_cap + 4);
}

template <int OP, bool F32, bool FILL, bool GT>
static void launch_tiled_gt(const SpmvPlan *plan, const SpmvArgs &a, hipStream_t s)
{
   int rowsum_elems, rp_cap;
   const size_t lds = tiled_lds_bytes(plan, rowsum_elems, rp_cap);
   const int unit = a.tile_perm ? 1 : (a.xcd_map > 0 ? 8 * a.xcd_map : 8);
   const int grid = ((plan->num_tiles + unit - 1) / unit) * unit;
   hipLaunchKernelGGL((spmv_tiled_kernel<OP, F32, FILL, GT>), dim3(grid), dim3(SPMV_THREADS), lds, s, a,
                      plan->d_tile_row, plan->d_tile_k, plan->num_tiles, plan->prod_elems, rowsum_elems, rp_cap);
}

template <int OP, int VF, bool FILL>
static void launch_xs(const SpmvPlan *plan, const SpmvArgs &a, hipStream_t s)
{
   int rowsum_elems, rp_cap;
   size_t lds = tiled_lds_bytes(plan, rowsum_elems, rp_cap);
   if (VF == VF_CODE) { lds = xs_dict_offset(plan->prod_elems, rowsum_elems, rp_cap) + sizeof(double) * (size_t) ((a.ndict + 1) & ~1); }
   const int unit = a.tile_perm ? 1 : (a.xcd_map > 0 ? 8 * a.xcd_map : 8);
   const int grid = ((plan->num_tiles + unit - 1) / unit) * unit;
   hipLaunchKernelGGL((spmv_xs_kernel<OP, VF, FILL>), dim3(grid), dim3(SPMV_THREADS), lds, s, a,
                      plan->d_tile_row, plan->d_tile_k, plan->d_xs_cnt, plan->d_xs_desc, plan->d_lidx,
                      plan->num_tiles, plan->prod_elems, rowsum_elems, rp_cap, plan->xs_launch_units);
}

static inline int sl_stage_elems(const SpmvPlan *plan) { return sl_stage_elems_of(plan->sl_launch_units, plan->d_sl_cls != nullptr); }
static inline size_t sl_table_bytes(const SpmvPlan *plan) { return plan->d_sl_cls ? sizeof(unsigned) * (size_t) plan->sl_classes * plan->sl_k : 0; }
static inline double sl_matrix_bytes(const SpmvPlan *plan, int ndict)
{
   const double blocks = (double) plan->sl_blocks, per_block = 4.0 * (XS_DESC + 4) + 8.0 * ndict + 4.0 * 72.0;
   if (plan->d_sl_cls) { return blocks * (per_block + (double) SPMV_THREADS + 4.0 * 3.0) + 4.0 * (double) plan->sl_class_total * plan->sl_k; }
   return blocks * (per_block + (double) SPMV_THREADS * plan->sl_k * 3.0) + 4.0 * ((double) plan->num_rows + 1.0);
}

template <int OP, int W, int KP>
static void launch_sl_form(const SpmvPlan *plan, const SpmvArgs &a, hipStream_t s)
{
   const int stage_elems = sl_stage_elems(plan);
   const size_t lds = sizeof(double) * (size_t) (stage_elems + ((a.ndict + 1) & ~1)) + sl_table_bytes(plan);
   const int grid = plan->d_sl_perm ? plan->sl_blocks : ((plan->sl_blocks + 63) / 64) * 64;
   if (plan->d_sl_cls)
   {
      hipLaunchKernelGGL((spmv_sl_kernel_cls<OP, W, KP>), dim3(grid), dim3(SPMV_THREADS), lds, s, a, plan->d_sl_desc, plan->d_sl_k0, plan->d_sl_fp,
                         plan->d_sl_perm, plan->d_sl_cls, plan->d_sl_tab, plan->d_sl_toff, plan->sl_blocks, plan->num_rows, plan->nnz, stage_elems);
      return;
   }
   hipLaunchKernelGGL((spmv_sl_kernel<OP, W, KP>), dim3(grid), dim3(SPMV_THREADS), lds, s, a, plan->d_sl_cnt, plan->d_sl_desc, plan->d_sl_k0,
                      plan->d_sl_fp, plan->d_sl_perm, plan->d_sl_data, plan->sl_blocks, plan->num_rows, plan->nnz, stage_elems);
}
template <int OP>
static void launch_sl(const SpmvPlan *plan, const SpmvArgs &a, hipStream_t s)
{
   if (plan->sl_w == 1) { launch_sl_form<OP, 1, 8>(plan, a, s); }
   else if (plan->sl_k == 8) { launch_sl_form<OP, 2, 8>(plan, a, s); }
   else { launch_sl_form<OP, 2, 16>(plan, a, s); }
}

template <int OP, int KP, bool F32>
static void launch_rs_form(const SpmvPlan *plan, const SpmvArgs &a, hipStream_t s)
{
   const int stage_elems = 2 * plan->rs_units + 8;
   const size_t lds = sizeof(double) * (size_t) (stage_elems + SPMV_THREADS);
   const int grid = plan->d_rs_perm ? plan->rs_blocks : ((plan->rs_blocks + 63) / 64) * 64;
   hipLaunchKernelGGL((spmv_rs_kernel<OP, KP, F32>), dim3(grid), dim3(SPMV_THREADS), lds, s, a, plan->d_rs_desc, plan->d_rs_perm, plan->d_rs_hdr,
                      plan->d_rs_meta, plan->d_rs_val, plan->d_rs_val32, plan->d_rs_idx, plan->rs_blocks, plan->num_rows, plan->rs_rows, plan->rs_w,
                      stage_elems);
}
template <int OP, bool F32>
static void launch_rs(const SpmvPlan *plan, const SpmvArgs &a, hipStream_t s)
{
   switch (plan->rs_kp)
   {
      case 8:  launch_rs_form<OP, 8, F32>(plan, a, s); break;
      case 16: launch_rs_form<OP, 16, F32>(plan, a, s); break;
      case 24: launch_rs_form<OP, 24, F32>(plan, a, s); break;
      default: launch_rs_form<OP, 32, F32>(plan, a, s); break;
   }
}
static inline bool takes_rs(const SpmvPlan *plan, const SpmvArgs &a)
{
   return plan->d_rs_val && a.variant == 2 && a.fill == HYPRE_SPMV_FILL_WHOLE && (((uintptr_t) a.x) & 15) == 0;
}

static inline bool takes_xs(const SpmvPlan *plan, const SpmvArgs &a)
{
   return plan->tiled && a.variant == 2 && a.gather_t && plan->d_lidx && (((uintptr_t) a.x) & 15) == 0;
}

template <int OP, bool F32, bool FILL>
static void launch_tiled(const SpmvPlan *plan, const SpmvArgs &a, hipStream_t s)
{
   if (!FILL && a.use_rs) { launch_rs<OP, F32>(plan, a, s); return; }
   if (takes_xs(plan, a))
   {
      if (a.Ac8 && !FILL && plan->has_slice_form()) { launch_sl<OP>(plan, a, s); }
      else if (a.Ac8) { launch_xs<OP, VF_CODE, FILL>(plan, a, s); }
      else { launch_xs<OP, F32 ? VF_F32 : VF_F64, FILL>(plan, a, s); }
      return;
   }
   if (a.gather_t) { launch_tiled_gt<OP, F32, FILL, true>(plan, a, s); }
   else { launch_tiled_gt<OP, F32, FILL, false>(plan, a, s); }
}

template <int OP>
static void launch_spmv_op(const SpmvPlan *plan, const SpmvArgs &a, hipStream_t s)
{
   const bool f32  = a.Aa32 != nullptr;
   const bool fill = a.fill != HYPRE_SPMV_FILL_WHOLE;
   if (plan->tiled)
   {
      if (f32) { if (fill) launch_tiled<OP, true, true>(plan, a, s); else launch_tiled<OP, true, false>(plan, a, s); }
      else     { if (fill) launch_tiled<OP, false, true>(plan, a, s); else launch_tiled<OP, false, false>(plan, a, s); }
   }
   else
   {
      int grid = (plan->num_rows + 3) / 4;
      if (grid > 4096) { grid = 4096; }
      if (grid < 1) { grid = 1; }
      dim3 g(grid), b(SPMV_THREADS);
      if (f32)
      {
         if (fill) hipLaunchKernelGGL((spmv_wave_kernel<OP, true, true>), g, b, 0, s, a, plan->num_rows);
         else      hipLaunchKernelGGL((spmv_wave_kernel<OP, true, false>), g, b, 0, s, a, plan->num_rows);
      }
      else
      {
         if (fill) hipLaunchKernelGGL((spmv_wave_kernel<OP, false, true>), g, b, 0, s, a, plan->num_rows);
         else      hipLaunchKernelGGL((spmv_wave_kernel<OP, false, false>), g, b, 0, s, a, plan->num_rows);
      }
   }
}

static void fill_plan_fields(SpmvArgs &a, const SpmvPlan *plan)
{
   a.last_quad = (plan->nnz > 0 ? (int) (plan->nnz - 1) : 0) & ~3;
   a.x_last = plan->num_cols > 0 ? plan->num_cols - 1 : 0;
   a.tile_perm = plan->d_tile_perm;
   a.tile_fp = plan->d_tile_fp;
   a.stale = plan->d_stale;
   a.nnz = plan->nnz;
}
static inline double rs_block_table_bytes(const SpmvPlan *plan) { return (double) plan->rs_blocks * (4.0 * (4 * RS_HDR + SPMV_THREADS + XS_DESC)); }

void launch_spmv(const SpmvPlan *plan, const SpmvArgs &args, SpmvOp op, hipStream_t s)
{
   if (plan->num_rows <= 0) { return; }
   SpmvArgs a = args;
   fill_plan_fields(a, plan);
   a.rot = const_cast<SpmvPlan *>(plan)->launches++;
   a.Ac8 = nullptr; a.dict = nullptr; a.ndict = 0; a.dict_rounded = 0;
   if (plan->d_codes && takes_xs(plan, a))
   {
      const bool rounded = handle().fp32_values || a.Aa32 != nullptr;
      a.Ac8 = plan->d_codes; a.ndict = plan->ndict;
      a.dict = rounded ? plan->d_dict32 : plan->d_dict;
      a.dict_rounded = rounded ? 1 : 0;
   }
   a.use_rs = takes_rs(plan, a) ? 1 : 0;
   if (a.use_rs && (handle().fp32_values || a.Aa32))
   {
      SpmvPlan *mp = const_cast<SpmvPlan *>(plan);
      if (!mp->d_rs_val32 && plan_alloc((void **) &mp->d_rs_val32, sizeof(float) * ((size_t) plan->nnz + 64), PLAN_SITE_ROWSLICE))
      {
         launch_f64_to_f32(plan->d_rs_val, mp->d_rs_val32, (size_t) plan->nnz, s);
      }
      if (mp->d_rs_val32) { a.Aa32 = mp->d_rs_val32; } else { a.use_rs = 0; }
   }
   if (handle().fp32_values && !a.Aa32 && !a.Ac8 && plan->nnz > 0)
   {
      SpmvPlan *mp = const_cast<SpmvPlan *>(plan);
      if (!mp->a32)
      {
         HIP_CHECK(hipMalloc((void **) &mp->a32, sizeof(float) * (((size_t) plan->nnz + 3) & ~(size_t) 3)));
         launch_f64_to_f32(plan->a, mp->a32, (size_t) plan->nnz, s);
      }
      a.Aa32 = mp->a32;
   }
   if (a.rowmap && op != OP_JACOBI_MAP) { hypre_error_w_msg(HYPRE_ERROR_ARG, "row map given to an operation that does not read it"); return; }
   {
      const double nz = (double) plan->nnz, nr = (double) plan->num_rows, vw = (a.Aa32 || a.dict_rounded) ? 4.0 : 8.0;
      const double xcols = 8.0 * std::min((double) plan->num_cols, nz);
      double rowb = 0.0;
      switch (op)
      {
         case OP_AXPBY:      rowb = 8.0 + ((a.beta != 0.0) ? 8.0 : 0.0); break;
         case OP_AXPBY_DIV:  rowb = 24.0 + ((a.beta != 0.0) ? 8.0 : 0.0); break;
         case OP_RESID_RD:   rowb = 16.0 + ((a.beta != 0.0) ? 8.0 : 0.0); break;
         case OP_TSGS_FIRST: rowb = 32.0 + ((a.beta != 0.0) ? 8.0 : 0.0); break;
         case OP_JACOBI:     rowb = 24.0; break;
         case OP_JACOBI_CF:  rowb = 28.0; break;
         case OP_JACOBI_MAP: rowb = 28.0 + (a.marker ? 4.0 : 0.0); break;
         case OP_TSGS:       rowb = 32.0; break;
      }
      const double rows_b = 4.0 * (nr + 1.0) + rowb * nr + xcols;
      const bool staged = takes_xs(plan, a);
      const bool slice = staged && a.Ac8 && a.fill == HYPRE_SPMV_FILL_WHOLE && plan->has_slice_form();
      double streamed;
      if (a.use_rs)
      {
         streamed = nz * (vw + 2.0) + rs_block_table_bytes(plan) + rowb * nr + xcols;
      }
      else if (slice)
      {
         streamed = sl_matrix_bytes(plan, a.ndict) + rowb * nr + xcols;
      }
      else if (staged)
      {
         streamed = nz * ((a.Ac8 ? 1.0 : vw) + 2.0) + rows_b + (double) plan->num_tiles * (4.0 * (XS_DESC + 6) + (a.Ac8 ? 8.0 * a.ndict : 0.0) + ((a.Ac8 || a.Aa32) ? 4.0 * 72.0 : 0.0));
      }
      else { streamed = nz * (vw + 4.0) + rows_b + (plan->tiled ? 8.0 * plan->num_tiles : 0.0); }
      account_bytes(nz * (vw + 4.0) + rows_b, streamed);
   }
   switch (op)
   {
      case OP_AXPBY:     launch_spmv_op<OP_AXPBY>(plan, a, s); break;
      case OP_AXPBY_DIV: launch_spmv_op<OP_AXPBY_DIV>(plan, a, s); break;
      case OP_RESID_RD:  launch_spmv_op<OP_RESID_RD>(plan, a, s); break;
      case OP_TSGS_FIRST: launch_spmv_op<OP_TSGS_FIRST>(plan, a, s); break;
      case OP_JACOBI:    launch_spmv_op<OP_JACOBI>(plan, a, s); break;
      case OP_JACOBI_CF: launch_spmv_op<OP_JACOBI_CF>(plan, a, s); break;
      case OP_JACOBI_MAP: launch_spmv_op<OP_JACOBI_MAP>(plan, a, s); break;
      case OP_TSGS:      launch_spmv_op<OP_TSGS>(plan, a, s); break;
   }
}

constexpr int MV_WIN = 2320;
struct MvLaunch
{
   int       stage_elems, rp_cap;
   size_t    lds;
   MvStrides st;
};
template <auto K>
static void allow_large_lds()
{
   static bool raised = false;
   if (raised) { return; }
   (void) hipFuncSetAttribute((const void *) K, hipFuncAttributeMaxDynamicSharedMemorySize, 160 * 1024);
   (void) hipGetLastError();
   raised = true;
}

template <int NV, bool CODED, int OP>
static void launch_xs_mv(const SpmvPlan *plan, const SpmvArgs &a, const MvLaunch &m, hipStream_t s)
{
   allow_large_lds<spmv_xs_mv_kernel<NV, CODED, OP>>();
   const int unit = a.tile_perm ? 1 : (a.xcd_map > 0 ? 8 * a.xcd_map : 8);
   const int grid = ((plan->num_tiles + unit - 1) / unit) * unit;
   const int threads = (plan->max_tile_rows > SPMV_THREADS && plan->max_tile_rows <= 320) ? 320 :
                       (plan->max_tile_rows > 320 ? MV_THREADS_MAX : SPMV_THREADS);
   hipLaunchKernelGGL((spmv_xs_mv_kernel<NV, CODED, OP>), dim3(grid), dim3(threads), m.lds, s, a,
                      plan->d_tile_row, plan->d_tile_k, plan->d_xs_cnt, plan->d_xs_desc, plan->d_lidx,
                      plan->num_tiles, m.stage_elems, MV_WIN, m.rp_cap, plan->xs_launch_units, m.st);
}

long &spmv_mv_launches() { static long n = 0; return n; }
template <int NV, int W, int KP, int OP>
static void launch_sl_mv(const SpmvPlan *plan, const SpmvArgs &a, const MvLaunch &m, hipStream_t s)
{
   const int grid = plan->d_sl_perm ? plan->sl_blocks : ((plan->sl_blocks + 63) / 64) * 64;
   if (plan->d_sl_cls)
   {
      allow_large_lds<spmv_sl_mv_kernel_cls<NV, W, KP, OP>>();
      hipLaunchKernelGGL((spmv_sl_mv_kernel_cls<NV, W, KP, OP>), dim3(grid), dim3(SPMV_THREADS), m.lds, s, a, plan->d_sl_desc, plan->d_sl_k0, plan->d_sl_fp,
                         plan->d_sl_perm, plan->d_sl_cls, plan->d_sl_tab, plan->d_sl_toff, plan->sl_blocks, plan->num_rows, plan->nnz, m.stage_elems,
                         m.st);
      return;
   }
   allow_large_lds<spmv_sl_mv_kernel<NV, W, KP, OP>>();
   hipLaunchKernelGGL((spmv_sl_mv_kernel<NV, W, KP, OP>), dim3(grid), dim3(SPMV_THREADS), m.lds, s, a, plan->d_sl_desc, plan->d_sl_k0,
                      plan->d_sl_fp, plan->d_sl_perm, plan->d_sl_data, plan->sl_blocks, plan->num_rows, plan->nnz, m.stage_elems, m.st);
}
template <int NV, int OP>
static void launch_sl_mv_nv(const SpmvPlan *plan, const SpmvArgs &a, const MvLaunch &m, hipStream_t s)
{
   if (plan->sl_w == 1) { launch_sl_mv<NV, 1, 8, OP>(plan, a, m, s); }
   else if (plan->sl_k == 8) { launch_sl_mv<NV, 2, 8, OP>(plan, a, m, s); }
   else { launch_sl_mv<NV, 2, 16, OP>(plan, a, m, s); }
}
static inline size_t sl_mv_lds_bytes(const SpmvPlan *plan, int nv, int ndict, int &stage_elems)
{
   stage_elems = sl_stage_elems(plan);
   return sizeof(double) * ((size_t) nv * stage_elems + (size_t) ((ndict + 1) & ~1)) + sl_table_bytes(plan);
}

template <int NV, int OP, int KP>
static void launch_rs_mv_form(const SpmvPlan *plan, const SpmvArgs &a, const MvLaunch &m, hipStream_t s)
{
   allow_large_lds<spmv_rs_mv_kernel<NV, OP, KP>>();
   const int grid = plan->d_rs_perm ? plan->rs_blocks : ((plan->rs_blocks + 63) / 64) * 64;
   hipLaunchKernelGGL((spmv_rs_mv_kernel<NV, OP, KP>), dim3(grid), dim3(SPMV_THREADS), m.lds, s, a, plan->d_rs_desc, plan->d_rs_perm, plan->d_rs_hdr,
                      plan->d_rs_meta, plan->d_rs_val, plan->d_rs_idx, plan->rs_blocks, plan->num_rows, plan->rs_rows, plan->rs_w, m.stage_elems,
                      m.st);
}
template <int NV, int OP>
static void launch_rs_mv(const SpmvPlan *plan, const SpmvArgs &a, const MvLaunch &m, hipStream_t s)
{
   switch (plan->rs_kp)
   {
      case 8:  launch_rs_mv_form<NV, OP, 8>(plan, a, m, s); break;
      case 16: launch_rs_mv_form<NV, OP, 16>(plan, a, m, s); break;
      case 24: launch_rs_mv_form<NV, OP, 24>(plan, a, m, s); break;
      default: launch_rs_mv_form<NV, OP, 32>(plan, a, m, s); break;
   }
}
static inline size_t rs_mv_lds_bytes(const SpmvPlan *plan, int nv, int &stage_elems)
{
   stage_elems = 2 * plan->rs_units + 8;
   return sizeof(double) * (size_t) nv * (size_t) (stage_elems + SPMV_THREADS);
}
static int rs_mv_columns()
{
   static const int c = [] { const char *e = getenv("HYPRE_AMD_SPMV_RS_MV_COLS"); const int v = e ? atoi(e) : 0; return (v >= 2 && v <= 4) ? v : 0; }();
   return c;
}

static inline size_t mv_lds_bytes(const SpmvPlan *plan, int nv, bool coded, int ndict, int &stage_elems, int &rp_cap)
{
   int rowsum_elems;
   (void) tiled_lds_bytes(plan, rowsum_elems, rp_cap);
   stage_elems = 2 * plan->xs_launch_units + 8;
   return sizeof(double) * (size_t) nv * stage_elems + (coded ? (size_t) MV_WIN : sizeof(double) * (size_t) MV_WIN) + sizeof(unsigned short) * (size_t) MV_WIN +
          sizeof(int) * (size_t) ((rp_cap + 4) & ~3) + (coded ? sizeof(double) * (size_t) ((ndict + 1) & ~1) : 0);
}

enum { MV_NONE = 0, MV_RS = 1, MV_SL = 2, MV_XS = 3 };
static int spmv_mv_form(const SpmvPlan *plan, const SpmvArgs &args, long xstride)
{
   const SpmvArgs &a = args;
   if (!plan->tiled || a.fill != HYPRE_SPMV_FILL_WHOLE || a.Aa32 || handle().fp32_values || a.rowmap || (xstride & 1) != 0) { return MV_NONE; }
   if (takes_rs(plan, a))
   {
      int stage_elems;
      return rs_mv_lds_bytes(plan, 2, stage_elems) <= (size_t) 160 * 1024 ? MV_RS : MV_NONE;
   }
   if (!takes_xs(plan, a) || !plan->d_tile_fp || !plan->d_stale) { return MV_NONE; }
   int stage_elems, rp_cap;
   if (plan->d_codes && plan->has_slice_form())
   {
      return sl_mv_lds_bytes(plan, 2, plan->ndict, stage_elems) <= (size_t) 160 * 1024 ? MV_SL : MV_NONE;
   }
   if (plan->max_row_nnz > SPMV_THREADS) { return MV_NONE; }
   if ((long long) plan->xs_tiles * 10 < (long long) plan->num_tiles * 9) { return MV_NONE; }
   return mv_lds_bytes(plan, 2, plan->d_codes != nullptr, plan->ndict, stage_elems, rp_cap) <= (size_t) 160 * 1024 ? MV_XS : MV_NONE;
}

template <int OP>
static void launch_mv_group(const SpmvPlan *plan, const SpmvArgs &c, int form, int g, bool coded, const MvLaunch &m, hipStream_t s)
{
   if (form == MV_RS)
   {
      switch (g)
      {
         case 2:  launch_rs_mv<2, OP>(plan, c, m, s); break;
         case 3:  launch_rs_mv<3, OP>(plan, c, m, s); break;
         default: launch_rs_mv<4, OP>(plan, c, m, s); break;
      }
   }
   else if (form == MV_SL)
   {
      switch (g)
      {
         case 2:  launch_sl_mv_nv<2, OP>(plan, c, m, s); break;
         case 3:  launch_sl_mv_nv<3, OP>(plan, c, m, s); break;
         default: launch_sl_mv_nv<4, OP>(plan, c, m, s); break;
// ... 113 lines not shown
```

### include/hypre_amd_seq_mv.h

```cpp
#ifndef HYPRE_AMD_SEQ_MV_H
#define HYPRE_AMD_SEQ_MV_H

#include "HYPRE_amd_utilities.h"

#ifdef __cplusplus
extern "C" {
#endif

typedef struct
{
   HYPRE_Int            *i;
   HYPRE_Int            *j;
   HYPRE_BigInt         *big_j;
   HYPRE_Int             num_rows;
   HYPRE_Int             num_cols;
   HYPRE_Int             num_nonzeros;
   hypre_int            *i_short;
   hypre_int            *j_short;
   HYPRE_Int             owns_data;
   HYPRE_Int             pattern_only;
   HYPRE_Complex        *data;
   HYPRE_Int            *rownnz;
   HYPRE_Int             num_rownnz;
   HYPRE_MemoryLocation  memory_location;
} hypre_CSRMatrix;

#define hypre_CSRMatrixData(matrix)            ((matrix) -> data)
#define hypre_CSRMatrixI(matrix)               ((matrix) -> i)
#define hypre_CSRMatrixJ(matrix)               ((matrix) -> j)
#define hypre_CSRMatrixBigJ(matrix)            ((matrix) -> big_j)
#define hypre_CSRMatrixNumRows(matrix)         ((matrix) -> num_rows)
#define hypre_CSRMatrixNumCols(matrix)         ((matrix) -> num_cols)
#define hypre_CSRMatrixNumNonzeros(matrix)     ((matrix) -> num_nonzeros)
#define hypre_CSRMatrixRownnz(matrix)          ((matrix) -> rownnz)
#define hypre_CSRMatrixNumRownnz(matrix)       ((matrix) -> num_rownnz)
#define hypre_CSRMatrixOwnsData(matrix)        ((matrix) -> owns_data)
#define hypre_CSRMatrixPatternOnly(matrix)     ((matrix) -> pattern_only)
#define hypre_CSRMatrixMemoryLocation(matrix)  ((matrix) -> memory_location)

typedef struct
{
   HYPRE_Complex        *data;
   HYPRE_Int             size;
   HYPRE_Int             component;
   HYPRE_Int             owns_data;
   HYPRE_MemoryLocation  memory_location;
   HYPRE_Int             num_vectors;
   HYPRE_Int             multivec_storage_method;
   HYPRE_Int             vecstride, idxstride;
} hypre_Vector;

#define hypre_VectorData(vector)                  ((vector) -> data)
#define hypre_VectorSize(vector)                  ((vector) -> size)
#define hypre_VectorComponent(vector)             ((vector) -> component)
#define hypre_VectorOwnsData(vector)              ((vector) -> owns_data)
#define hypre_VectorMemoryLocation(vector)        ((vector) -> memory_location)
#define hypre_VectorNumVectors(vector)            ((vector) -> num_vectors)
#define hypre_VectorMultiVecStorageMethod(vector) ((vector) -> multivec_storage_method)
#define hypre_VectorVectorStride(vector)          ((vector) -> vecstride)
#define hypre_VectorIndexStride(vector)           ((vector) -> idxstride)

#define HYPRE_SPMV_FILL_STRICT_LOWER -2
#define HYPRE_SPMV_FILL_LOWER        -1
#define HYPRE_SPMV_FILL_WHOLE         0
#define HYPRE_SPMV_FILL_UPPER         1
#define HYPRE_SPMV_FILL_STRICT_UPPER  2

hypre_CSRMatrix *hypre_CSRMatrixCreate(HYPRE_Int num_rows, HYPRE_Int num_cols, HYPRE_Int num_nonzeros);
HYPRE_Int hypre_CSRMatrixInitialize_v2(hypre_CSRMatrix *matrix, HYPRE_Int bigInit,
                                       HYPRE_MemoryLocation memory_location);
HYPRE_Int hypre_CSRMatrixInitialize(hypre_CSRMatrix *matrix);
HYPRE_Int hypre_CSRMatrixDestroy(hypre_CSRMatrix *matrix);
HYPRE_Int hypre_CSRMatrixSetRownnz(hypre_CSRMatrix *matrix);
HYPRE_Int hypre_CSRMatrixMigrate(hypre_CSRMatrix *A, HYPRE_MemoryLocation memory_location);
hypre_CSRMatrix *hypre_CSRMatrixClone_v2(hypre_CSRMatrix *A, HYPRE_Int copy_data,
                                         HYPRE_MemoryLocation memory_location);
HYPRE_Int hypre_CSRMatrixTranspose(hypre_CSRMatrix *A, hypre_CSRMatrix **AT, HYPRE_Int data);
HYPRE_Int hypre_CSRMatrixReorder(hypre_CSRMatrix *A);

hypre_Vector *hypre_SeqVectorCreate(HYPRE_Int size);
hypre_Vector *hypre_SeqMultiVectorCreate(HYPRE_Int size, HYPRE_Int num_vectors);
HYPRE_Int hypre_SeqVectorInitialize_v2(hypre_Vector *vector, HYPRE_MemoryLocation memory_location);
HYPRE_Int hypre_SeqVectorInitialize(hypre_Vector *vector);
HYPRE_Int hypre_SeqVectorDestroy(hypre_Vector *vector);
HYPRE_Int hypre_SeqVectorMigrate(hypre_Vector *x, HYPRE_MemoryLocation memory_location);
hypre_Vector *hypre_SeqVectorCloneDeep_v2(hypre_Vector *x, HYPRE_MemoryLocation memory_location);
hypre_Vector *hypre_SeqVectorCloneDeep(hypre_Vector *x);

HYPRE_Int hypre_CSRMatrixMatvecOutOfPlace(HYPRE_Complex alpha, hypre_CSRMatrix *A, hypre_Vector *x,
                                          HYPRE_Complex beta, hypre_Vector *b, hypre_Vector *y,
                                          HYPRE_Int offset);
HYPRE_Int hypre_CSRMatrixMatvec(HYPRE_Complex alpha, hypre_CSRMatrix *A, hypre_Vector *x,
                                HYPRE_Complex beta, hypre_Vector *y);
HYPRE_Int hypre_CSRMatrixMatvecT(HYPRE_Complex alpha, hypre_CSRMatrix *A, hypre_Vector *x,
                                 HYPRE_Complex beta, hypre_Vector *y);
HYPRE_Int hypre_CSRMatrixMatvecDevice(HYPRE_Int trans, HYPRE_Complex alpha, hypre_CSRMatrix *A,
                                      hypre_Vector *x, HYPRE_Complex beta, hypre_Vector *b,
                                      hypre_Vector *y, HYPRE_Int offset);
HYPRE_Int hypre_CSRMatrixSpMVDevice(HYPRE_Int trans, HYPRE_Complex alpha, hypre_CSRMatrix *B,
                                    hypre_Vector *x, HYPRE_Complex beta, hypre_Vector *y,
                                    HYPRE_Int fill);

HYPRE_Int hypre_amd_CSRMatrixInvalidatePlan(hypre_CSRMatrix *A);
HYPRE_Int hypre_amd_CSRMatrixVerifyPlan(hypre_CSRMatrix *A);
HYPRE_Int hypre_amd_CSRMatrixSetImmutable(hypre_CSRMatrix *A, HYPRE_Int on);
HYPRE_Int hypre_amd_SetMixedPrecisionValues(HYPRE_Int on);
HYPRE_Int hypre_amd_CSRMatrixPlanForm(hypre_CSRMatrix *A);
HYPRE_Int hypre_amd_PlanTestFailAlloc(HYPRE_Int site, HYPRE_Int nth);
HYPRE_Int hypre_amd_CSRMatrixSortRows(hypre_CSRMatrix *A, HYPRE_Int keep_first);
HYPRE_Int hypre_amd_SpmvSetBandPolicy(HYPRE_Int enabled, HYPRE_Int min_tiles, HYPRE_Int force);
HYPRE_Int hypre_amd_SpmvSetVariant(HYPRE_Int variant, HYPRE_Int unused);
HYPRE_Int hypre_amd_SpmvSetValueCodes(HYPRE_Int on);
HYPRE_Int hypre_amd_SpmvSetSliceForm(HYPRE_Int on);
HYPRE_Int hypre_amd_SpmvSetSliceClasses(HYPRE_Int on);
HYPRE_Int hypre_amd_SpmvSetRowSlices(HYPRE_Int mode);
HYPRE_Int hypre_amd_SpmvSetFusedMultivectors(HYPRE_Int on);
HYPRE_Int hypre_amd_SpmvFusedMultivectorLaunches(void);
HYPRE_Int hypre_amd_CSRMatrixPlanRowSlices(hypre_CSRMatrix *A, HYPRE_Int *rows_per_block, HYPRE_Int *entries_per_lane);
HYPRE_Int hypre_amd_CSRMatrixPlanSliceForm(hypre_CSRMatrix *A);
HYPRE_Int hypre_amd_CSRMatrixPlanSliceClasses(hypre_CSRMatrix *A);
HYPRE_Int hypre_amd_CSRMatrixPlanSliceClassHistogram(hypre_CSRMatrix *A, HYPRE_Int *hist, HYPRE_Int *blocks, HYPRE_BigInt *total);
HYPRE_Int hypre_amd_CSRMatrixPlanValueCodes(hypre_CSRMatrix *A);
HYPRE_Int hypre_amd_CSRMatrixPlanStaging(hypre_CSRMatrix *A, HYPRE_Int *num_tiles, HYPRE_Real *mean_pieces);
HYPRE_Int hypre_amd_CSRMatrixPlanInfo(hypre_CSRMatrix *A, HYPRE_Int *num_tiles, HYPRE_Int *band);

HYPRE_Int hypre_SeqVectorSetConstantValues(hypre_Vector *v, HYPRE_Complex value);
HYPRE_Int hypre_SeqVectorCopy(hypre_Vector *x, hypre_Vector *y);
HYPRE_Int hypre_SeqVectorScale(HYPRE_Complex alpha, hypre_Vector *y);
HYPRE_Int hypre_SeqVectorAxpy(HYPRE_Complex alpha, hypre_Vector *x, hypre_Vector *y);
HYPRE_Int hypre_SeqVectorAxpyz(HYPRE_Complex alpha, hypre_Vector *x, HYPRE_Complex beta,
                               hypre_Vector *y, hypre_Vector *z);
HYPRE_Real hypre_SeqVectorInnerProd(hypre_Vector *x, hypre_Vector *y);
HYPRE_Int hypre_SeqVectorElmdivpy(hypre_Vector *x, hypre_Vector *b, hypre_Vector *y);
HYPRE_Int hypre_SeqVectorElmdivpyMarked(hypre_Vector *x, hypre_Vector *b, hypre_Vector *y,
                                        HYPRE_Int *marker, HYPRE_Int marker_val);
HYPRE_Int hypre_SeqVectorSetConstantValuesDevice(hypre_Vector *v, HYPRE_Complex value);
HYPRE_Int hypre_SeqVectorScaleDevice(HYPRE_Complex alpha, hypre_Vector *y);
HYPRE_Int hypre_SeqVectorAxpyDevice(HYPRE_Complex alpha, hypre_Vector *x, hypre_Vector *y);
HYPRE_Int hypre_SeqVectorAxpyzDevice(HYPRE_Complex alpha, hypre_Vector *x, HYPRE_Complex beta,
                                     hypre_Vector *y, hypre_Vector *z);
HYPRE_Real hypre_SeqVectorInnerProdDevice(hypre_Vector *x, hypre_Vector *y);
HYPRE_Int hypre_SeqVectorElmdivpyDevice(hypre_Vector *x, hypre_Vector *b, hypre_Vector *y,
                                        HYPRE_Int *marker, HYPRE_Int marker_val);
HYPRE_Int hypreDevice_IVAXPY(HYPRE_Int n, HYPRE_Complex *a, HYPRE_Complex *x, HYPRE_Complex *y);
HYPRE_Int hypreDevice_IVAXPYMarked(HYPRE_Int n, HYPRE_Complex *a, HYPRE_Complex *x, HYPRE_Complex *y,
                                   HYPRE_Int *marker, HYPRE_Int marker_val);
HYPRE_Int hypreDevice_DiagScaleVector2(HYPRE_Int num_vectors, HYPRE_Int num_rows,
                                       HYPRE_Complex *diag, HYPRE_Complex *x, HYPRE_Complex beta,
                                       HYPRE_Complex *y, HYPRE_Complex *z, HYPRE_Int computeY);

#ifdef __cplusplus
}
#endif
#endif
```

Measured before the change: 9.430 billion DOF/s.

## Add wide 16-bit value-code SpMV form for matrices with many distinct values

```diff
diff --git a/hypre_amd/binding.py b/hypre_amd/binding.py
--- a/hypre_amd/binding.py
+++ b/hypre_amd/binding.py
@@ -195,6 +195,7 @@
     "hypre_amd_CSRMatrixPlanInfo": (Int, [CSRp, IntP, IntP]),
     "hypre_amd_CSRMatrixPlanStaging": (Int, [CSRp, IntP, RealP]),
     "hypre_amd_SpmvSetValueCodes": (Int, [Int]),
+    "hypre_amd_SpmvSetWideCodes": (Int, [Int]),
     "hypre_amd_SpmvSetSliceForm": (Int, [Int]),
     "hypre_amd_CSRMatrixPlanSliceForm": (Int, [CSRp]),
     "hypre_amd_SpmvSetSliceClasses": (Int, [Int]),
diff --git a/hypre_amd/csrc/internal.hpp b/hypre_amd/csrc/internal.hpp
--- a/hypre_amd/csrc/internal.hpp
+++ b/hypre_amd/csrc/internal.hpp
@@ -108,6 +108,12 @@
    int            sl_classes = 0;
    long long      sl_class_total = 0;
    bool has_slice_form() const { return d_sl_data != nullptr || d_sl_cls != nullptr; }
+   unsigned *d_wc_data = nullptr;
+   double   *d_wc_table = nullptr;
+   int      *d_wc_desc = nullptr;
+   int       wc_ndict = 0, wc_kp = 0, wc_blocks = 0, wc_units = 0;
+   bool      wc_lds = false;
+   unsigned  codes_epoch = 0;
    int             rs_w = 0, rs_rows = 0, rs_kp = 0;
    int             rs_blocks = 0, rs_units = 0;
    int            *d_rs_desc = nullptr;
@@ -135,7 +141,7 @@
 bool is_owned(const hypre_CSRMatrix *A);
 bool plan_verify(hypre_CSRMatrix *A);
 enum PlanAllocSite { PLAN_SITE_TILES = 1, PLAN_SITE_XS = 2, PLAN_SITE_CODES = 3, PLAN_SITE_SLICE = 4, PLAN_SITE_ROWSLICE = 5, PLAN_SITE_SLICE_CLASSES = 6,
-                     PLAN_SITE_MV_LEVELS = 7 };
+                     PLAN_SITE_MV_LEVELS = 7, PLAN_SITE_WIDE = 8 };
 bool plan_alloc(void **ptr, size_t bytes, int site);
 void plan_free(void *ptr);
 inline void verify_par_plans(hypre_ParCSRMatrix *A)
@@ -236,6 +242,8 @@
 bool device_value_codes(const double *Aa, size_t nnz, unsigned char **codes_out, double **dict_out, double **dict32_out, int *ndict_out,
                         hipStream_t s);
 bool device_build_slice_form(SpmvPlan *p, const hypre_CSRMatrix *A, hipStream_t s);
+bool device_build_wide_codes(SpmvPlan *p, const hypre_CSRMatrix *A, hipStream_t s);
+bool &spmv_wide_codes();
 bool device_build_row_slices(SpmvPlan *p, const hypre_CSRMatrix *A, hipStream_t s);
 int  &spmv_row_slices();
 bool &spmv_slice_classes();
diff --git a/hypre_amd/csrc/seq_mv.cpp b/hypre_amd/csrc/seq_mv.cpp
--- a/hypre_amd/csrc/seq_mv.cpp
+++ b/hypre_amd/csrc/seq_mv.cpp
@@ -129,6 +129,8 @@
 static unsigned long long g_plan_generation = 1;
 unsigned long long plan_generation() { return g_plan_generation; }
 void bump_plan_generation() { g_plan_generation++; }
+static unsigned g_codes_epoch = 1;
+static void codes_switch_changed() { g_codes_epoch++; g_plan_generation++; }
 
 namespace {
 struct StaleSlots
@@ -210,6 +212,7 @@
    if (p->d_sl_cls) { HIP_CHECK(hipFree(p->d_sl_cls)); }
    if (p->d_sl_tab) { HIP_CHECK(hipFree(p->d_sl_tab)); }
    if (p->d_sl_toff) { HIP_CHECK(hipFree(p->d_sl_toff)); }
+   plan_free(p->d_wc_data); plan_free(p->d_wc_table); plan_free(p->d_wc_desc);
    for (void *q : {(void *) p->d_rs_desc, (void *) p->d_rs_perm, (void *) p->d_rs_hdr, (void *) p->d_rs_meta, (void *) p->d_rs_val,
                    (void *) p->d_rs_val32, (void *) p->d_rs_idx}) { plan_free(q); }
    if (p->AT) { hypre_CSRMatrixDestroy(p->AT); }
@@ -318,17 +321,20 @@
    }
    p->prod_elems = std::max(p->prod_elems, 2 * p->xs_launch_units + 8);
    if (p->d_codes && spmv_slice_form()) { device_build_slice_form(p, A, s); }
+   if (!p->d_codes && p->owned && p->max_row_nnz <= 8 && spmv_value_codes() && spmv_wide_codes() && spmv_slice_form()) { device_build_wide_codes(p, A, s); }
 }
 
 SpmvPlan *get_plan(hypre_CSRMatrix *A)
 {
    auto &t = plan_table();
    auto it = t.find(A);
+   hypre_CSRMatrix *kept_AT = nullptr, *kept_L = nullptr;
    if (it != t.end())
    {
       SpmvPlan *p = it->second;
       const bool flagged = p->h_stale && __atomic_load_n(p->h_stale, __ATOMIC_RELAXED) != 0;
-      if (!flagged && p->i == A->i && p->j == A->j && p->a == A->data && p->nnz == A->num_nonzeros &&
+      const bool switched = p->owned && p->tiled && p->max_row_nnz <= 8 && p->codes_epoch != g_codes_epoch;
+      if (!flagged && !switched && p->i == A->i && p->j == A->j && p->a == A->data && p->nnz == A->num_nonzeros &&
           p->num_rows == A->num_rows && p->num_cols == A->num_cols)
       {
          return p;
@@ -341,13 +347,16 @@
          drop_gs_schedule(A);
          drop_mc_plan(A);
       }
+      else if (switched && p->i == A->i && p->j == A->j && p->a == A->data && p->nnz == A->num_nonzeros) { std::swap(kept_AT, p->AT); std::swap(kept_L, p->Lstrict); }
       free_plan(p);
       t.erase(it);
    }
    SpmvPlan *p = new SpmvPlan();
+   p->AT = kept_AT; p->Lstrict = kept_L;
    p->i = A->i; p->j = A->j; p->a = A->data;
    p->num_rows = A->num_rows; p->num_cols = A->num_cols; p->nnz = A->num_nonzeros;
    p->owned = is_owned(A);
+   p->codes_epoch = g_codes_epoch;
    hipStream_t s = stream();
    if (A->num_rows > 0 && A->num_nonzeros > 0)
    {
@@ -404,6 +413,12 @@
 bool &spmv_value_codes()
 {
    static bool on = [] { const char *e = getenv("HYPRE_AMD_SPMV_VALUE_CODES"); return !(e && atoi(e) == 0); }();
+   return on;
+}
+
+bool &spmv_wide_codes()
+{
+   static bool on = [] { const char *e = getenv("HYPRE_AMD_SPMV_WIDE_CODES"); return !(e && atoi(e) == 0); }();
    return on;
 }
 
@@ -487,8 +502,14 @@
 
 extern "C" HYPRE_Int hypre_amd_SpmvSetValueCodes(HYPRE_Int on)
 {
-   if (on >= 0) { hamd::spmv_value_codes() = on != 0; }
-   return hypre_error_flag;
+   if (on >= 0 && hamd::spmv_value_codes() != (on != 0)) { hamd::spmv_value_codes() = on != 0; hamd::codes_switch_changed(); }
+   return hypre_error_flag;
+}
+
+extern "C" HYPRE_Int hypre_amd_SpmvSetWideCodes(HYPRE_Int on)
+{
+   if (on >= 0 && hamd::spmv_wide_codes() != (on != 0)) { hamd::spmv_wide_codes() = on != 0; hamd::codes_switch_changed(); }
+   return hamd::spmv_wide_codes() ? 1 : 0;
 }
 
 extern "C" HYPRE_Int hypre_amd_SpmvSetSliceForm(HYPRE_Int on)
@@ -548,14 +569,14 @@
 {
    if (A->memory_location != HYPRE_MEMORY_DEVICE) { return 0; }
    hamd::SpmvPlan *p = hamd::get_plan(A);
-   return p->has_slice_form() ? p->sl_w : 0;
+   return p->has_slice_form() ? p->sl_w : (p->d_wc_data ? 1 : 0);
 }
 
 extern "C" HYPRE_Int hypre_amd_CSRMatrixPlanValueCodes(hypre_CSRMatrix *A)
 {
    if (A->memory_location != HYPRE_MEMORY_DEVICE) { return 0; }
    hamd::SpmvPlan *p = hamd::get_plan(A);
-   return p->d_codes ? p->ndict : 0;
+   return p->d_codes ? p->ndict : (p->d_wc_data ? p->wc_ndict : 0);
 }
 
 extern "C" HYPRE_Int hypre_amd_CSRMatrixPlanInfo(hypre_CSRMatrix *A, HYPRE_Int *num_tiles, HYPRE_Int *band)
@@ -633,7 +654,7 @@
    if (!p->tiled) { return 0; }
    if (p->d_rs_val) { return 5; }
    if (!p->d_lidx) { return 1; }
-   if (p->has_slice_form()) { return 4; }
+   if (p->has_slice_form() || p->d_wc_data) { return 4; }
    if (p->d_codes) { return 3; }
    return 2;
 }
diff --git a/hypre_amd/csrc/spmv_kernels.hip b/hypre_amd/csrc/spmv_kernels.hip
--- a/hypre_amd/csrc/spmv_kernels.hip
+++ b/hypre_amd/csrc/spmv_kernels.hip
@@ -1405,6 +1405,105 @@
    spmv_sl_mv_body<NV, W, KP, true, OP>(p, sl_desc, sl_k0, sl_fp, sl_perm, st, blocks, num_rows, nnz, stage_elems, ms);
 }
 
+constexpr int WC_CAP = 65536;
+constexpr int WC_LDS_CAP = 2048;
+constexpr int WC_NB = 4;
+template <int OP, int KP, int NB, bool LTAB>
+__global__ __launch_bounds__(SPMV_THREADS * NB)
+void spmv_slw_kernel(SpmvArgs p, const int *__restrict__ wc_desc, const unsigned *__restrict__ wc_data, const double *__restrict__ table,
+                     int ntab, int blocks, int num_rows, int stage_elems)
+{
+   extern __shared__ __align__(16) unsigned char smem_raw[];
+   const int tid = threadIdx.x, lane = tid & 63;
+   const int wq = __builtin_amdgcn_readfirstlane(tid >> 6), wave = wq & 3, grp = wq >> 2;
+   double *xs = reinterpret_cast<double *>(smem_raw) + (size_t) grp * stage_elems;
+   double *tabl = reinterpret_cast<double *>(smem_raw) + (size_t) NB * stage_elems;
+
+   const int g8 = (int) blockIdx.x >> 3, c8 = (int) blockIdx.x & 7;
+   const int block = ((g8 >> 3) * 64 + c8 * 8 + (g8 & 7)) * NB + grp;
+   const bool valid = block < blocks;
+   if (NB == 1 && !valid) { return; }
+   const int bl = valid ? block : blocks - 1;
+   const int r = bl * SPMV_THREADS + (tid & (SPMV_THREADS - 1));
+   constexpr int H = KP / 2;
+   unsigned cw[H], lw[H];
+   const unsigned *sd = wc_data + ((size_t) (bl * 4 + wave) * (size_t) KP) * 64 + lane;
+#pragma unroll
+   for (int w = 0; w < H; w++) { cw[w] = sd[w * 64]; }
+#pragma unroll
+   for (int w = 0; w < H; w++) { lw[w] = sd[(H + w) * 64]; }
+   const RowOps ops = load_row_ops<OP>(p, max(min(r, num_rows - 1), 0));
+   const XPieces pc = wave_x_pieces(wc_desc, bl, wave);
+   asm volatile("" :: "s"(wc_desc), "s"(wc_data) : "memory");
+   if (valid) { stage_x_pieces<1>(p.x, 0, xs, 0, pc, lane); }
+   double a[KP];
+   if constexpr (LTAB)
+   {
+      for (int c = wq; 128 * c < ntab; c += 4 * NB)
+      {
+         if (128 * c + 2 * lane < ntab)
+         {
+            __builtin_amdgcn_global_load_lds((const __attribute__((address_space(1))) void *) (table + 128 * c + 2 * lane),
+                                             (__attribute__((address_space(3))) void *) (tabl + 128 * c), 16, 0, 0);
+         }
+      }
+   }
+   else
+   {
+#pragma unroll
+      for (int j = 0; j < KP; j++) { a[j] = table[(cw[j >> 1] >> (16 * (j & 1))) & 0xffffu]; }
+   }
+   __syncthreads();
+
+   const int mylen = (int) ((lw[0] >> 12) & 0xfu);
+   double sum = 0.0;
+#pragma unroll
+   for (int j = 0; j < KP; j++)
+   {
+      const unsigned li = (lw[j >> 1] >> (16 * (j & 1))) & 0xfffu;
+      if constexpr (LTAB) { a[j] = tabl[(cw[j >> 1] >> (16 * (j & 1))) & 0xffffu]; }
+      {
+#pragma clang fp contract(off)
+         const double pr = a[j] * xs[li];
+         if (j < mylen) { sum = sum + pr; }
+      }
+   }
+   if (valid && r < num_rows) { row_epilogue<OP>(p, r, sum, ops); }
+}
+
+__global__ __launch_bounds__(SPMV_THREADS)
+void slw_pack_kernel(const int *__restrict__ Ai, const unsigned long long *__restrict__ vals, const unsigned short *__restrict__ lidx,
+                     const unsigned long long *__restrict__ table, int ntab, int num_rows, int kp, unsigned *__restrict__ data,
+                     int *__restrict__ fail)
+{
+   const int block = blockIdx.x, tid = threadIdx.x, lane = tid & 63, wave = tid >> 6;
+   const int r = block * SPMV_THREADS + tid;
+   const int rs = r < num_rows ? Ai[r] : 0, re = r < num_rows ? Ai[r + 1] : 0;
+   const int len = re - rs, h = kp / 2;
+   bool bad = len < 0 || len > kp;
+   unsigned *out = data + ((size_t) (block * 4 + wave) * (size_t) kp) * 64 + lane;
+   for (int w = 0; w < h; w++)
+   {
+      unsigned cword = 0, lword = 0;
+      for (int q = 0; q < 2; q++)
+      {
+         const int j = 2 * w + q;
+         if (j >= len || bad) { continue; }
+         const unsigned long long v = vals[rs + j];
+         int lo = 0, hi = ntab;
+         while (lo < hi) { const int mid = (lo + hi) >> 1; if (table[mid] < v) { lo = mid + 1; } else { hi = mid; } }
+         const unsigned li = lidx[rs + j];
+         if (lo >= ntab || table[lo] != v || li > 0xfffu) { bad = true; continue; }
+         cword |= (unsigned) lo << (16 * q);
+         lword |= li << (16 * q);
+      }
+      if (w == 0) { lword |= (unsigned) (bad ? 0 : len) << 12; }
+      out[w * 64] = cword;
+      out[(h + w) * 64] = lword;
+   }
+   if (bad) { atomicOr(fail, 1); }
+}
+
 __global__ void sl_block_starts_kernel(const int *__restrict__ Ai, int num_rows, int R, int blocks, int *__restrict__ k0)
 {
    const int b = blockIdx.x * blockDim.x + threadIdx.x;
@@ -2156,11 +2255,13 @@
 
 constexpr int DICT_SLOTS = 4 * DICT_CAP;
 constexpr unsigned long long DICT_EMPTY = ~0ull;
+template <int CAP = DICT_CAP>
 __device__ __forceinline__ unsigned dict_hash(unsigned long long v)
 {
    v ^= v >> 33; v *= 0xff51afd7ed558ccdull; v ^= v >> 29;
-   return (unsigned) v & (DICT_SLOTS - 1);
-}
+   return (unsigned) v & (4 * CAP - 1);
+}
+template <int CAP>
 __global__ __launch_bounds__(256)
 void dict_collect_kernel(const unsigned long long *__restrict__ vals, size_t n, unsigned long long *table, int *count)
 {
@@ -2169,12 +2270,12 @@
    {
       const unsigned long long v = vals[k];
       if (v == last) { continue; }
-      if (v == DICT_EMPTY || __hip_atomic_load(count, __ATOMIC_RELAXED, __HIP_MEMORY_SCOPE_AGENT) > DICT_CAP)
-      {
-         __hip_atomic_store(count, DICT_CAP + 1, __ATOMIC_RELAXED, __HIP_MEMORY_SCOPE_AGENT);
+      if (v == DICT_EMPTY || __hip_atomic_load(count, __ATOMIC_RELAXED, __HIP_MEMORY_SCOPE_AGENT) > CAP)
+      {
+         __hip_atomic_store(count, CAP + 1, __ATOMIC_RELAXED, __HIP_MEMORY_SCOPE_AGENT);
          return;
       }
-      unsigned slot = dict_hash(v);
+      unsigned slot = dict_hash<CAP>(v);
       for (;;)
       {
          unsigned long long cur = __hip_atomic_load(table + slot, __ATOMIC_RELAXED, __HIP_MEMORY_SCOPE_AGENT);
@@ -2184,8 +2285,8 @@
             if (cur == DICT_EMPTY) { atomicAdd(count, 1); break; }
          }
          if (cur == v) { break; }
-         if (__hip_atomic_load(count, __ATOMIC_RELAXED, __HIP_MEMORY_SCOPE_AGENT) > DICT_CAP) { return; }
-         slot = (slot + 1) & (DICT_SLOTS - 1);
+         if (__hip_atomic_load(count, __ATOMIC_RELAXED, __HIP_MEMORY_SCOPE_AGENT) > CAP) { return; }
+         slot = (slot + 1) & (4 * CAP - 1);
       }
       last = v;
    }
@@ -2220,12 +2321,12 @@
    const unsigned long long *bits = reinterpret_cast<const unsigned long long *>(Aa);
    int count = 0;
    const size_t head = std::min<size_t>(nnz, 16384);
-   hipLaunchKernelGGL(dict_collect_kernel, dim3((unsigned) ((head + 255) / 256)), dim3(256), 0, s, bits, head, d_table, d_count);
+   hipLaunchKernelGGL(dict_collect_kernel<DICT_CAP>, dim3((unsigned) ((head + 255) / 256)), dim3(256), 0, s, bits, head, d_table, d_count);
    HIP_CHECK(hipMemcpyAsync(&count, d_count, sizeof(int), hipMemcpyDeviceToHost, s));
    HIP_CHECK(hipStreamSynchronize(s));
    if (count > DICT_CAP) { plan_free(d_table); return false; }
    int grid = (int) std::min<size_t>((nnz + 255) / 256, (size_t) 8 * handle().num_cus);
-   if (nnz > head) { hipLaunchKernelGGL(dict_collect_kernel, dim3(grid), dim3(256), 0, s, bits, nnz, d_table, d_count); }
+   if (nnz > head) { hipLaunchKernelGGL(dict_collect_kernel<DICT_CAP>, dim3(grid), dim3(256), 0, s, bits, nnz, d_table, d_count); }
    std::vector<unsigned long long> table(DICT_SLOTS);
    HIP_CHECK(hipMemcpyAsync(&count, d_count, sizeof(int), hipMemcpyDeviceToHost, s));
    HIP_CHECK(hipMemcpyAsync(table.data(), d_table, sizeof(unsigned long long) * DICT_SLOTS, hipMemcpyDeviceToHost, s));
@@ -2268,6 +2369,90 @@
    return true;
 }
 
+bool device_build_wide_codes(SpmvPlan *p, const hypre_CSRMatrix *A, hipStream_t s)
+{
+   const int K = p->max_row_nnz, n = A->num_rows, nnz = A->num_nonzeros;
+   if (K < 1 || K > 8 || n < 1 || nnz < 1) { return false; }
+   const int kp = K <= 4 ? 4 : 8;
+   const long long blocks_ll = ((long long) n + SPMV_THREADS - 1) / SPMV_THREADS;
+   if (4.0 * kp * (double) n > 0.5 * 12.0 * (double) nnz || blocks_ll > (1LL << 26)) { return false; }
+   const int blocks = (int) blocks_ll;
+   static const int table_mode = [] { const char *e = getenv("HYPRE_AMD_SPMV_WIDE_TABLE"); return e ? atoi(e) : 0; }();
+   static const bool verbose = getenv("HYPRE_AMD_PLAN_VERBOSE") != nullptr;
+   constexpr int SLOTS = 4 * WC_CAP;
+   unsigned long long *d_hash = nullptr;
+   int *d_k0 = nullptr, *d_cnt = nullptr, *d_desc = nullptr, *d_fail = nullptr;
+   unsigned short *d_li = nullptr;
+   unsigned *d_data = nullptr;
+   double *d_table = nullptr;
+   auto fail = [&](const char *why) -> bool
+   {
+      HIP_CHECK(hipStreamSynchronize(s));
+      for (void *q : {(void *) d_hash, (void *) d_k0, (void *) d_cnt, (void *) d_desc, (void *) d_fail, (void *) d_li, (void *) d_data, (void *) d_table}) { plan_free(q); }
+      if (verbose) { fprintf(stderr, "[plan] %d x %d: no wide codes (%s)\n", n, A->num_cols, why); }
+      return false;
+   };
+   if (!plan_alloc((void **) &d_hash, sizeof(unsigned long long) * SLOTS + sizeof(int) * 4, PLAN_SITE_WIDE)) { return fail("table"); }
+   int *d_count = reinterpret_cast<int *>(d_hash + SLOTS);
+   HIP_CHECK(hipMemsetAsync(d_hash, 0xff, sizeof(unsigned long long) * SLOTS, s));
+   HIP_CHECK(hipMemsetAsync(d_count, 0, sizeof(int) * 4, s));
+   const unsigned long long *bits = reinterpret_cast<const unsigned long long *>(A->data);
+   const int grid = (int) std::min<size_t>(((size_t) nnz + 255) / 256, (size_t) 8 * handle().num_cus);
+   hipLaunchKernelGGL(dict_collect_kernel<WC_CAP>, dim3(grid), dim3(256), 0, s, bits, (size_t) nnz, d_hash, d_count);
+   int count = 0;
+   HIP_CHECK(hipMemcpyAsync(&count, d_count, sizeof(int), hipMemcpyDeviceToHost, s));
+   HIP_CHECK(hipStreamSynchronize(s));
+   if (count > WC_CAP || count <= 0) { return fail("more than 65536 values"); }
+   if (3LL * count > (long long) nnz) { return fail("values used less than three times on average"); }
+   std::vector<unsigned long long> slots((size_t) SLOTS), vals;
+   HIP_CHECK(hipMemcpyAsync(slots.data(), d_hash, sizeof(unsigned long long) * SLOTS, hipMemcpyDeviceToHost, s));
+   HIP_CHECK(hipStreamSynchronize(s));
+   vals.reserve((size_t) count);
+   for (unsigned long long v : slots) { if (v != DICT_EMPTY) { vals.push_back(v); } }
+   std::sort(vals.begin(), vals.end());
+   if ((int) vals.size() != count) { (void) fail("count"); hypre_error_w_msg(HYPRE_ERROR_GENERIC, "value table: count and contents disagree"); return false; }
+   const size_t tab_elems = (((size_t) count + 1) & ~(size_t) 1) + 2;
+   vals.resize(tab_elems, 0ull);
+   const size_t nl = ((size_t) nnz + 15) & ~(size_t) 7;
+   if (!plan_alloc((void **) &d_table, sizeof(double) * tab_elems, PLAN_SITE_WIDE) ||
+       !plan_alloc((void **) &d_k0, sizeof(int) * ((size_t) blocks + 1), PLAN_SITE_WIDE) ||
+       !plan_alloc((void **) &d_cnt, sizeof(int) * (size_t) blocks, PLAN_SITE_WIDE) ||
+       !plan_alloc((void **) &d_desc, sizeof(int) * (size_t) blocks * XS_DESC, PLAN_SITE_WIDE) ||
+       !plan_alloc((void **) &d_li, sizeof(unsigned short) * nl, PLAN_SITE_WIDE)) { return fail("tables"); }
+   HIP_CHECK(hipMemcpyAsync(d_table, vals.data(), sizeof(double) * tab_elems, hipMemcpyHostToDevice, s));
+   hipLaunchKernelGGL(sl_block_starts_kernel, dim3((blocks + 256) / 256), dim3(256), 0, s, A->i, n, SPMV_THREADS, blocks, d_k0);
+   HIP_CHECK(hipMemsetAsync(d_li, 0, sizeof(unsigned short) * nl, s));
+   launch_build_xs(A->j, d_k0, blocks, d_cnt, d_desc, d_li, s);
+   std::vector<int> cnt((size_t) blocks), k0((size_t) blocks + 1);
+   HIP_CHECK(hipMemcpyAsync(cnt.data(), d_cnt, sizeof(int) * (size_t) blocks, hipMemcpyDeviceToHost, s));
+   HIP_CHECK(hipMemcpyAsync(k0.data(), d_k0, sizeof(int) * ((size_t) blocks + 1), hipMemcpyDeviceToHost, s));
+   HIP_CHECK(hipStreamSynchronize(s));
+   int units = 0;
+   for (int b = 0; b < blocks; b++)
+   {
+      const int c = cnt[(size_t) b];
+      if ((c & 0xff) == 0 && k0[(size_t) b + 1] > k0[(size_t) b]) { return fail("a block cannot be staged"); }
+      units = std::max(units, c >> 8);
+   }
+   const size_t stage_bytes = 8 * (size_t) (2 * units + 8);
+   if (stage_bytes > 40 * 1024) { return fail("LDS"); }
+   const bool lds_table = table_mode == 1 && count <= WC_LDS_CAP && WC_NB * stage_bytes + 8 * tab_elems <= 64 * 1024;
+   if (!plan_alloc((void **) &d_data, sizeof(unsigned) * (size_t) blocks * 4 * (size_t) kp * 64, PLAN_SITE_WIDE) ||
+       !plan_alloc((void **) &d_fail, sizeof(int), PLAN_SITE_WIDE)) { return fail("words"); }
+   HIP_CHECK(hipMemsetAsync(d_fail, 0, sizeof(int), s));
+   hipLaunchKernelGGL(slw_pack_kernel, dim3(blocks), dim3(SPMV_THREADS), 0, s, A->i, bits, d_li, reinterpret_cast<const unsigned long long *>(d_table),
+                      count, n, kp, d_data, d_fail);
+   int failed = 0;
+   HIP_CHECK(hipMemcpyAsync(&failed, d_fail, sizeof(int), hipMemcpyDeviceToHost, s));
+   HIP_CHECK(hipStreamSynchronize(s));
+   if (failed) { return fail("packing"); }
+   plan_free(d_hash); plan_free(d_k0); plan_free(d_cnt); plan_free(d_li); plan_free(d_fail);
+   p->d_wc_data = d_data; p->d_wc_table = d_table; p->d_wc_desc = d_desc;
+   p->wc_ndict = count; p->wc_kp = kp; p->wc_blocks = blocks; p->wc_units = units; p->wc_lds = lds_table;
+   if (verbose) { fprintf(stderr, "[plan] %d x %d: wide codes, %d values, %d words a row, %d blocks, %d units, table %s\n", n, A->num_cols, count, kp, blocks, units, lds_table ? "in LDS" : "gathered"); }
+   return true;
+}
+
 static inline size_t tiled_lds_bytes(const SpmvPlan *plan, int &rowsum_elems, int &rp_cap)
 {
    static int fit = -1;
@@ -2334,6 +2519,37 @@
    else { launch_sl_form<OP, 2, 16>(plan, a, s); }
 }
 
+static inline bool takes_wide(const SpmvPlan *plan, const SpmvArgs &a, SpmvOp op)
+{
+   return plan->d_wc_data && (op == OP_AXPBY || op == OP_AXPBY_DIV) && a.variant == 2 && a.gather_t && a.fill == HYPRE_SPMV_FILL_WHOLE &&
+          !a.Aa32 && !handle().fp32_values && !a.rowmap && (((uintptr_t) a.x) & 15) == 0;
+}
+static inline double wide_matrix_bytes(const SpmvPlan *plan)
+{
+   const double blocks = (double) plan->wc_blocks, table = 8.0 * plan->wc_ndict;
+   return blocks * (4.0 * XS_DESC + 4.0 * SPMV_THREADS * plan->wc_kp) + (plan->wc_lds ? table * std::ceil(blocks / WC_NB) : table);
+}
+template <int OP, int KP>
+static void launch_slw_form(const SpmvPlan *plan, const SpmvArgs &a, hipStream_t s)
+{
+   const int stage_elems = 2 * plan->wc_units + 8;
+   if (plan->wc_lds)
+   {
+      const int wgs = (plan->wc_blocks + WC_NB - 1) / WC_NB;
+      const size_t lds = sizeof(double) * ((size_t) WC_NB * stage_elems + (((size_t) plan->wc_ndict + 1) & ~(size_t) 1));
+      hipLaunchKernelGGL((spmv_slw_kernel<OP, KP, WC_NB, true>), dim3(((wgs + 63) / 64) * 64), dim3(SPMV_THREADS * WC_NB), lds, s, a, plan->d_wc_desc,
+                         plan->d_wc_data, plan->d_wc_table, plan->wc_ndict, plan->wc_blocks, plan->num_rows, stage_elems);
+      return;
+   }
+   hipLaunchKernelGGL((spmv_slw_kernel<OP, KP, 1, false>), dim3(((plan->wc_blocks + 63) / 64) * 64), dim3(SPMV_THREADS), sizeof(double) * (size_t) stage_elems,
+                      s, a, plan->d_wc_desc, plan->d_wc_data, plan->d_wc_table, plan->wc_ndict, plan->wc_blocks, plan->num_rows, stage_elems);
+}
+static void launch_slw(const SpmvPlan *plan, const SpmvArgs &a, SpmvOp op, hipStream_t s)
+{
+   if (op == OP_AXPBY) { if (plan->wc_kp == 4) { launch_slw_form<OP_AXPBY, 4>(plan, a, s); } else { launch_slw_form<OP_AXPBY, 8>(plan, a, s); } }
+   else { if (plan->wc_kp == 4) { launch_slw_form<OP_AXPBY_DIV, 4>(plan, a, s); } else { launch_slw_form<OP_AXPBY_DIV, 8>(plan, a, s); } }
+}
+
 template <int OP, int KP, bool F32>
 static void launch_rs_form(const SpmvPlan *plan, const SpmvArgs &a, hipStream_t s)
 {
@@ -2434,6 +2650,7 @@
       a.dict = rounded ? plan->d_dict32 : plan->d_dict;
       a.dict_rounded = rounded ? 1 : 0;
    }
+   const bool wide = !plan->d_codes && takes_wide(plan, a, op);
    a.use_rs = takes_rs(plan, a) ? 1 : 0;
    if (a.use_rs && (handle().fp32_values || a.Aa32))
    {
@@ -2474,7 +2691,8 @@
       const bool staged = takes_xs(plan, a);
       const bool slice = staged && a.Ac8 && a.fill == HYPRE_SPMV_FILL_WHOLE && plan->has_slice_form();
       double streamed;
-      if (a.use_rs)
+      if (wide) { streamed = wide_matrix_bytes(plan) + rowb * nr + xcols; }
+      else if (a.use_rs)
       {
          streamed = nz * (vw + 2.0) + rs_block_table_bytes(plan) + rowb * nr + xcols;
       }
@@ -2489,6 +2707,7 @@
       else { streamed = nz * (vw + 4.0) + rows_b + (plan->tiled ? 8.0 * plan->num_tiles : 0.0); }
       account_bytes(nz * (vw + 4.0) + rows_b, streamed);
    }
+   if (wide) { launch_slw(plan, a, op, s); return; }
    switch (op)
    {
       case OP_AXPBY:     launch_spmv_op<OP_AXPBY>(plan, a, s); break;
diff --git a/include/hypre_amd_seq_mv.h b/include/hypre_amd_seq_mv.h
--- a/include/hypre_amd_seq_mv.h
+++ b/include/hypre_amd_seq_mv.h
@@ -111,6 +111,7 @@
 HYPRE_Int hypre_amd_SpmvSetBandPolicy(HYPRE_Int enabled, HYPRE_Int min_tiles, HYPRE_Int force);
 HYPRE_Int hypre_amd_SpmvSetVariant(HYPRE_Int variant, HYPRE_Int unused);
 HYPRE_Int hypre_amd_SpmvSetValueCodes(HYPRE_Int on);
+HYPRE_Int hypre_amd_SpmvSetWideCodes(HYPRE_Int on);
 HYPRE_Int hypre_amd_SpmvSetSliceForm(HYPRE_Int on);
 HYPRE_Int hypre_amd_SpmvSetSliceClasses(HYPRE_Int on);
 HYPRE_Int hypre_amd_SpmvSetRowSlices(HYPRE_Int mode);
```

After: 9.191 billion DOF/s. 0.975x the previous value.
